# rayandrew/indonesian-image-captioning

Measured on AMD Instinct MI355X. Metric: images/sec (train step, SCN+Attention, bs32/GPU), higher is better.
Workload: dtype f32; 1 GPU; attention_scn decoder (emb/att/factor/dec=512, 1000 tags, V=10000, T=51) + ResNet-152 fine-tune, synthetic tags, bs=32/GPU, 256x256 images, fp32; global_batch=32, parallelism=dp1, call_sequence=harness: encoder(imgs, pooled=False) -> decoder(None, ..., prepool=trunk map)

## Files before the change

include/scnattn.h:

```cpp
#ifndef SCNATTN_H
#define SCNATTN_H

#include <stddef.h>
#include <stdint.h>

#ifdef __cplusplus
extern "C" {
#endif

#define SCNATTN_VERSION 109

int scnattn_version(void);
const char* scnattn_last_error(void);
int scnattn_set_option(const char* name, int value);
int scnattn_profile_collect(double* out6);

typedef struct {
    int B;
    int P;
    int E;
    int A;
    int D;
    int F;
    int M;
// ... 357 lines not shown
    int32_t H, W, C;
    int32_t tab_h;
    int32_t tab_v;
    int32_t reserved;
} scnattn_image_desc;
long scnattn_resize_table_ints(int in_size, int out_size);
int scnattn_u8_resize_bilinear(void* stream, const uint8_t* src, long src_bytes, const scnattn_image_desc* desc_host,
                               const scnattn_image_desc* desc_dev, int N, const int32_t* taps, long taps_len, int OH,
                               int OW, const float* lut, void* dst, int dst_kind, int channels_last);
int scnattn_u8_resize_taps(void* stream, const uint8_t* src, long src_bytes, const scnattn_image_desc* desc_host,
                           const scnattn_image_desc* desc_dev, int N, const int32_t* taps_host, const int32_t* taps_dev,
                           long taps_len, int OH, int OW, const float* lut, void* dst, int dst_kind, int channels_last);
#define SCNATTN_OVERLAY_MAX_MAP 32
#define SCNATTN_OVERLAY_MAX_OUT 1024
int scnattn_attn_strips(int OH);
int scnattn_attn_expand(void* stream, const float* alphas, int n_maps, int h, int w, const float* Mv, const float* Mh,
                        int OH, int OW, float* S, float* lohi, float* partial);
int scnattn_attn_overlay(void* stream, const float* alphas, int n_maps, int h, int w, const float* Mv, const float* Mh,
                         int OH, int OW, const float* S, const float* partial, const uint8_t* img, int n_img,
                         const int32_t* img_index_host, const int32_t* img_index_dev, const float* beta, uint8_t* out);
#define SCNATTN_TEXT_MAX_LEN 128
#define SCNATTN_TEXT_MAX_REFS 32
#define SCNATTN_TEXT_CIDER_MAX_TOKEN 65534
int scnattn_text_max_len(void);
int scnattn_text_ngram_stats(void* stream, int N, int R, const int32_t* hyp, int Lh, const int32_t* hyp_len, const int32_t* ref,
                             int Lr, const int32_t* ref_len, const int32_t* skip_hyp, int n_skip_hyp, const int32_t* skip_ref,
                             int n_skip_ref, int32_t* stats);
int scnattn_text_lcs(void* stream, int N, int R, const int32_t* hyp, int Lh, const int32_t* hyp_len, const int32_t* ref, int Lr,
                     const int32_t* ref_len, const int32_t* skip_hyp, int n_skip_hyp, const int32_t* skip_ref, int n_skip_ref,
                     int32_t* lcs, double* score, double* mean);
int scnattn_text_ref_keys(void* stream, int n, int N, int R, const int32_t* ref, int Lr, const int32_t* ref_len,
                          const int32_t* skip_ref, int n_skip_ref, int64_t* keys, int32_t* flag);
int scnattn_text_cider(void* stream, int N, int R, const int32_t* hyp, int Lh, const int32_t* hyp_len, const int32_t* ref,
                       int Lr, const int32_t* ref_len, const int32_t* skip_hyp, int n_skip_hyp, const int32_t* skip_ref,
                       int n_skip_ref, const int64_t* table_keys, const int32_t* table_df, const long* table_off, long n_images,
                       double* score, double* mean, int32_t* flag);
int scnattn_bn_workspace_floats(int C);
int scnattn_bn_stats(void* stream, int R, int C, const void* x, int bf16, float eps, float momentum, float* partial,
                     float* mean, float* invstd, float* run_mean, float* run_var);
int scnattn_bn_apply(void* stream, int R, int C, const void* z, const void* res, int bf16, const float* mean,
                     const float* invstd, const float* gamma, const float* beta, int relu, void* y);
int scnattn_bn_bwd(void* stream, int R, int C, const void* dy, const void* y, const void* z, int bf16,
                   const float* mean, const float* invstd, const float* gamma, const float* beta, int relu, int train,
                   float* partial, float* dbeta, float* dgamma, void* dz, void* dres);
typedef struct scnattn_conv_extra {
    int pro;
    int epi;
    const float* pro_ss;
    float* stat_partial; const float* stat_shift;
    const float* ez; const float* emean; const float* einvstd; const float* egamma; const float* ebeta; long ldz;
    int stride, Hi, Wi, Ho, Wo;
    int force_split;
    int force_mi;
} scnattn_conv_extra;
int scnattn_cgemm(void* stream, int transA, int transB, int M, int N, int K, float alpha, const float* A, long lda,
                  const float* B, long ldb, float beta, float* C, long ldc, const float* bias, const float* rowmask,
                  int batch, long strideA, long strideB, long strideC, float* ws, long ws_floats,
                  const scnattn_conv_extra* ex);
int scnattn_cgemm_row_tiles(int M);
int scnattn_conv1x1_fwd(void* stream, int R, int Cin, int Cout, const float* x, const float* w, float* y,
                        const scnattn_conv_extra* ex, float* ws, long ws_floats);
int scnattn_conv1x1_dgrad(void* stream, int R, int Cin, int Cout, const float* dy, const float* w, int w_transposed,
                          float beta, float* dx, const scnattn_conv_extra* ex, float* ws, long ws_floats);
int scnattn_conv1x1_wgrad(void* stream, int R, int Cin, int Cout, const float* dy, const float* x, float* dw,
                          const scnattn_conv_extra* ex, float* ws, long ws_floats);
int scnattn_conv3x3_fwd(void* stream, int N, int Hi, int Wi, int Cin, int Cout, int stride, const float* x,
                        const float* w, float* y, const scnattn_conv_extra* ex, float* ws, long ws_floats);
int scnattn_conv3x3_dgrad(void* stream, int N, int Hi, int Wi, int Cin, int Cout, const float* dy, const float* w,
                          float* dx, const scnattn_conv_extra* ex, float* ws, long ws_floats);
int scnattn_conv3x3_dgrad_strided(void* stream, int N, int Hi, int Wi, int Cin, int Cout, int stride, const float* dy,
                                  const float* w, float* dx, float* ws, long ws_floats);
int scnattn_conv3x3_wgrad(void* stream, int N, int Hi, int Wi, int Cin, int Cout, int stride, const float* dy,
                          const float* x, float* dw, float* ws, long ws_floats, int k_slices);
typedef struct scnattn_bn_eval {
    const float* gamma; const float* beta; const float* mean; const float* var; float eps;
    const float* res; long ldres;
    int relu;
} scnattn_bn_eval;
int scnattn_conv1x1_fwd_bn_eval(void* stream, int R, int Cin, int Cout, const float* x, const float* w, float* y,
                                const scnattn_bn_eval* bn, const scnattn_conv_extra* ex, float* ws, long ws_floats);
int scnattn_conv3x3_fwd_bn_eval(void* stream, int N, int Hi, int Wi, int Cin, int Cout, int stride, const float* x,
                                const float* w, float* y, const scnattn_bn_eval* bn, const scnattn_conv_extra* ex,
                                float* ws, long ws_floats);
int scnattn_stem_tiles(int N, int H, int W);
int scnattn_stem_conv7(void* stream, int N, int H, int W, const float* x, long sn, long sc, long sh, long sw,
                       const float* w, long wn, long wc, long wh, long ww, float* z, float* stat_partial,
                       const float* stat_shift);
int scnattn_stem_bn_relu_maxpool(void* stream, int N, int Hz, int Wz, int C, const float* z, const float* ss, void* out,
                                 int out_bf16);
int scnattn_cgemm_stat_ld(int M);
int scnattn_bn_finalize(void* stream, long R, int C, const float* partial, int ldp, int nchunk, const float* shift,
                        float eps, float momentum, float* mean, float* invstd, float* run_mean, float* run_var,
                        const float* gamma, const float* beta, float* ss_out);
int scnattn_bn_apply_fin(void* stream, long R, int C, const void* z, const void* res, int bf16, const float* partial, int ldp,
                         int nchunk, const float* shift, float eps, float momentum, const float* gamma, const float* beta,
                         int relu, void* y, float* mean, float* invstd, float* run_mean, float* run_var, float* ss_out);
int scnattn_bn_bwd_reduce(void* stream, int R, int C, const void* dy, const void* y, const void* z, int bf16, const float* mean,
                          const float* invstd, int relu, float* partial, int ldp_cap, void* gout, int* nchunk_out);
int scnattn_bn_bwd_dx_fin(void* stream, long R, int C, const void* g, const void* z, int bf16, const float* mean,
                          const float* invstd, const float* gamma, const float* partial, int ldp, int nchunk, float* dbeta,
                          float* dgamma, void* dz);

typedef struct scnattn_weight_desc {
    const float* src; void* dst; void* dst_t; int cout, taps, cin, pad;
} scnattn_weight_desc;
int scnattn_bf16_weights(void* stream, int n, const scnattn_weight_desc* desc, const int* tile_prefix, int total_tiles);
int scnattn_cgemm16(void* stream, int M, int N, int K, const void* A, long lda, const void* B, long ldb, float beta, void* C,
                    long ldc, int out_bf16, float* ws, long ws_floats, const scnattn_conv_extra* ex);
int scnattn_conv3x3_fwd16(void* stream, int N, int Hi, int Wi, int Cin, int Cout, int stride, const void* x, const void* w,
                          void* y, const scnattn_conv_extra* ex, float* ws, long ws_floats);
int scnattn_conv3x3_dgrad16(void* stream, int N, int Hi, int Wi, int Cin, int Cout, int stride, const void* dy, const void* wt,
                            void* dx, const scnattn_conv_extra* ex, float* ws, long ws_floats);
typedef struct scnattn_bn_eval16 {
    const float* gamma; const float* beta; const float* mean; const float* var; float eps;
    const void* res; long ldres;
    int relu;
} scnattn_bn_eval16;
int scnattn_conv1x1_fwd_bn_eval16(void* stream, int R, int Cin, int Cout, const void* x, const void* w, void* y,
                                  const scnattn_bn_eval16* bn, const scnattn_conv_extra* ex, float* ws, long ws_floats);
int scnattn_conv3x3_fwd_bn_eval16(void* stream, int N, int Hi, int Wi, int Cin, int Cout, int stride, const void* x,
                                  const void* w, void* y, const scnattn_bn_eval16* bn, const scnattn_conv_extra* ex,
                                  float* ws, long ws_floats);
int scnattn_wgrad16_3x3(void* stream, int N, int H, int W, int Cin, int Cout, const void* dy, const void* x, float* dw,
                        float* ws, long ws_floats, int k_slices);
int scnattn_wgrad16_rows(void* stream, int R, int Cin, int Cout, const void* dy, const void* x, long src_rows, float* dw,
                         long ldo, int gs, int gHi, int gWi, int gHo, int gWo, int goh, int gow, float* ws, long ws_floats,
                         int k_slices);
typedef struct scnattn_block16 {
    int N, Cin, Hi, Wi, p, stride, has_down, pad;
    const float* gamma[4]; const float* beta[4]; float* run_mean[4]; float* run_var[4]; const float* shift[4];
    float eps[4], momentum[4];
    const void* w[4]; const void* wt[4];
    float* ws; long ws_floats; float* part; float* bnpart; long bnpart_floats;
    const void* x; void* save; float* stats;
    const void* dout; void* tmp; float* dgb; float* dw[4]; int need_dx, pad2;
    void* side_stream; float* side_ws; long side_ws_floats;
} scnattn_block16;
int scnattn_block16_sizes(const scnattn_block16* b, long* save_elems, long* out_offset, long* stats_floats, long* tmp_elems,
                          long* dgb_floats);
int scnattn_block16_fwd(void* stream, const scnattn_block16* b);
int scnattn_block16_bwd(void* stream, const scnattn_block16* b, void** dx_out, void** dxd_out);
int scnattn_bn_stats_fold(void* stream, int R, int C, const void* x, float eps, float momentum, float* partial,
                          float* mean, float* invstd, float* run_mean, float* run_var, const float* gamma,
                          const float* beta, float* ss_out);

enum { SCNATTN_PLAN_NONE = 0, SCNATTN_PLAN_CGEMM, SCNATTN_PLAN_SGEMM, SCNATTN_PLAN_SKINNY, SCNATTN_PLAN_CGEMM16,
// ... 48 lines not shown
```

indonesian-image-captioning_amd/csrc/api.cpp:

```cpp
#include <hip/hip_runtime.h>
#include <cstdarg>
#include <cstdio>
#include <cstring>
#include "../../include/scnattn.h"
#include "common.h"
#include "kernels.h"

namespace scn {

static thread_local char g_err[512] = "";

void set_error(const char* fmt, ...) {
    va_list ap;
    va_start(ap, fmt);
    vsnprintf(g_err, sizeof(g_err), fmt, ap);
    va_end(ap);
}
const char* last_error() { return g_err; }

thread_local LaunchPlan* t_plan_out = nullptr;

extern int g_ksplit_scale;
extern int g_profile;
extern int g_attn_depth;
// ... 473 lines not shown
                             const float* enc, float inv_temp, int t0, int n_steps, float* ws) {
    return score_steps(ST(stream), d, K, max_steps, want_alpha, w, enc, inv_temp, t0, n_steps, ws);
}
int scnattn_rollout_score(void* stream, int N, int K, int V, const float* logits, long ld, float inv_temp, int t, int max_steps,
                          void* const* state, const int32_t* target_t, int32_t* rank_t, int32_t* best_t) {
    RolloutState s;
    SCN_TRY(rollout_state_of("scnattn_rollout_score", N, K, max_steps, state, s));
    return rollout_score(ST(stream), N, K, V, logits, ld, inv_temp, t, target_t, rank_t, best_t, s);
}

int scnattn_seq_workspace(const scnattn_dims* d, const scnattn_pool* pool, size_t* saved_bytes, size_t* scratch_bytes) {
    return seq_workspace(d, pool, saved_bytes, scratch_bytes);
}

int scnattn_seq_fwd(void* stream, const scnattn_dims* d, const scnattn_params* w, const float* enc,
                    const float* tags, const int64_t* caps, const int32_t* dl_dev, const int32_t* bt_host,
                    const float* drop_mask, float* saved, float* scratch, float* preds, float* alphas,
                    const scnattn_pool* pool) {
    return seq_fwd(ST(stream), d, w, enc, tags, caps, dl_dev, bt_host, drop_mask, saved, scratch, preds, alphas, pool);
}

int scnattn_seq_bwd(void* stream, const scnattn_dims* d, const scnattn_params* w, const float* enc,
                    const float* tags, const int64_t* caps, const int32_t* dl_dev, const int32_t* bt_host,
                    const float* drop_mask, const float* saved, float* scratch, const float* dpreds,
                    const float* dalphas, const scnattn_params* g, float* denc, float* dtags,
                    const scnattn_pool* pool) {
    return seq_bwd(ST(stream), d, w, enc, tags, caps, dl_dev, bt_host, drop_mask, saved, scratch, dpreds, dalphas, g,
                   denc, dtags, pool);
}

int scnattn_sgemm(void* stream, int transA, int transB, int M, int N, int K, float alpha, const float* A,
                  long lda, const float* B, long ldb, float beta, float* C, long ldc, const float* bias,
                  const float* rowmask, int batch, long strideA, long strideB, long strideC) {
    return sgemm(ST(stream), transA != 0, transB != 0, M, N, K, alpha, A, lda, B, ldb, beta, C, ldc, bias, rowmask,
                 batch < 1 ? 1 : batch, strideA, strideB, strideC);
}

int scnattn_sgemm_ws(void* stream, int transA, int transB, int M, int N, int K, float alpha, const float* A,
                     long lda, const float* B, long ldb, float beta, float* C, long ldc, const float* bias,
                     const float* rowmask, int batch, long strideA, long strideB, long strideC, float* ws,
                     long ws_floats) {
    return sgemm_ws(ST(stream), transA != 0, transB != 0, M, N, K, alpha, A, lda, B, ldb, beta, C, ldc, bias, rowmask,
                    batch < 1 ? 1 : batch, strideA, strideB, strideC, ws, ws ? ws_floats : 0);
}

static ConvExtra to_extra(const scnattn_conv_extra* e) {
    ConvExtra x;
    if (!e) return x;
    x.pro = e->pro; x.epi = e->epi; x.pro_ss = e->pro_ss;
    x.stat_partial = e->stat_partial; x.stat_shift = e->stat_shift;
    x.ez = e->ez; x.emean = e->emean; x.einvstd = e->einvstd; x.egamma = e->egamma; x.ebeta = e->ebeta; x.ldz = e->ldz;
    x.stride = e->stride < 1 ? 1 : e->stride; x.Hi = e->Hi; x.Wi = e->Wi; x.Ho = e->Ho; x.Wo = e->Wo;
    x.force_split = e->force_split; x.force_mi = e->force_mi;
    return x;
}

int scnattn_cgemm(void* stream, int transA, int transB, int M, int N, int K, float alpha, const float* A, long lda,
                  const float* B, long ldb, float beta, float* C, long ldc, const float* bias, const float* rowmask,
                  int batch, long strideA, long strideB, long strideC, float* ws, long ws_floats,
                  const scnattn_conv_extra* ex) {
    const ConvExtra x = to_extra(ex);
    return cgemm(ST(stream), transA != 0, transB != 0, M, N, K, alpha, A, lda, B, ldb, beta, C, ldc, bias, rowmask,
                 batch < 1 ? 1 : batch, strideA, strideB, strideC, ws, ws ? ws_floats : 0, ex ? &x : nullptr);
}

int scnattn_cgemm_row_tiles(int M) { return cgemm_row_tiles(M); }

int scnattn_conv1x1_fwd(void* stream, int R, int Cin, int Cout, const float* x, const float* w, float* y,
                        const scnattn_conv_extra* ex, float* ws, long ws_floats) {
    const ConvExtra e = to_extra(ex);
    SCN_ARG(!ex || ex->pro != 2, "conv1x1_fwd: prologue must be on the input (pro = 1)");
    return cgemm(ST(stream), false, true, R, Cout, Cin, 1.f, x, Cin, w, Cin, 0.f, y, Cout, nullptr, nullptr, 1, 0, 0, 0,
                 ws, ws ? ws_floats : 0, ex ? &e : nullptr);
}

int scnattn_conv1x1_dgrad(void* stream, int R, int Cin, int Cout, const float* dy, const float* w, int w_transposed,
                          float beta, float* dx, const scnattn_conv_extra* ex, float* ws, long ws_floats) {
    const ConvExtra e = to_extra(ex);
    SCN_ARG(!ex || (ex->pro == 0 && ex->stride <= 1), "conv1x1_dgrad: no prologue / stride here");
    if (w_transposed)
        return cgemm(ST(stream), false, true, R, Cin, Cout, 1.f, dy, Cout, w, Cout, beta, dx, Cin, nullptr, nullptr, 1, 0,
                     0, 0, ws, ws ? ws_floats : 0, ex ? &e : nullptr);
    return cgemm(ST(stream), false, false, R, Cin, Cout, 1.f, dy, Cout, w, Cin, beta, dx, Cin, nullptr, nullptr, 1, 0, 0,
                 0, ws, ws ? ws_floats : 0, ex ? &e : nullptr);
}

int scnattn_conv1x1_wgrad(void* stream, int R, int Cin, int Cout, const float* dy, const float* x, float* dw,
                          const scnattn_conv_extra* ex, float* ws, long ws_floats) {
    ConvExtra e = to_extra(ex);
    SCN_ARG(!ex || (ex->pro != 1 && ex->epi == 0), "conv1x1_wgrad: prologue must be on the input (pro = 2), no epilogue");
    return cgemm(ST(stream), true, false, Cout, Cin, R, 1.f, dy, Cout, x, Cin, 0.f, dw, Cin, nullptr, nullptr, 1, 0, 0, 0,
                 ws, ws ? ws_floats : 0, ex ? &e : nullptr);
}

static void set_c3(ConvExtra& e, int mode, int c, int N, int Hi, int Wi, int stride) {
    e.c3 = mode; e.c3c = c;
    e.Hi = Hi; e.Wi = Wi; e.Ho = (Hi - 1) / stride + 1; e.Wo = (Wi - 1) / stride + 1; e.stride = stride;
    e.c3_src_rows = mode == 4 ? (long)N * e.Ho * e.Wo : (long)N * Hi * Wi;
}

int scnattn_conv3x3_fwd(void* stream, int N, int Hi, int Wi, int Cin, int Cout, int stride, const float* x,
                        const float* w, float* y, const scnattn_conv_extra* ex, float* ws, long ws_floats) {
    SCN_ARG(N > 0 && Hi > 0 && Wi > 0 && stride >= 1, "conv3x3_fwd: geometry");
    ConvExtra e = to_extra(ex);
    set_c3(e, 1, Cin, N, Hi, Wi, stride);
    return cgemm(ST(stream), false, true, N * e.Ho * e.Wo, Cout, 9 * Cin, 1.f, x, Cin, w, 9L * Cin, 0.f, y, Cout, nullptr,
                 nullptr, 1, 0, 0, 0, ws, ws ? ws_floats : 0, &e);
}

static int bn_eval_extra(const char* who, int Cin, int Cout, const scnattn_bn_eval* bn, const scnattn_conv_extra* ex,
                         ConvExtra* e) {
    if (!bn) { set_error("%s: invalid argument: bn is NULL", who); return -1; }
    if (ex && (ex->pro != 0 || ex->epi != 0)) { set_error("%s: invalid argument: ex carries geometry only (pro = epi = 0)", who); return -1; }
    if (!(bn->gamma && bn->beta && bn->mean && bn->var)) { set_error("%s: invalid argument: null BatchNorm parameter / statistic", who); return -1; }
    if (Cin <= 0 || Cout <= 0 || Cin % 16 || Cout % 16) { set_error("%s: invalid argument: Cin and Cout must be positive multiples of 16", who); return -1; }
    if (!(aligned16(bn->gamma) && aligned16(bn->beta) && aligned16(bn->mean) && aligned16(bn->var))) {
        set_error("%s: invalid argument: BatchNorm vectors must be 16-byte aligned", who); return -1;
    }
    if (bn->res && (!aligned16(bn->res) || bn->ldres % 4 || bn->ldres < Cout)) {
        set_error("%s: invalid argument: res must be 16-byte aligned with ldres %% 4 == 0 and ldres >= Cout", who); return -1;
    }
    if (ex) {
        e->stride = ex->stride < 1 ? 1 : ex->stride; e->Hi = ex->Hi; e->Wi = ex->Wi; e->Ho = ex->Ho; e->Wo = ex->Wo;
        e->force_split = ex->force_split; e->force_mi = ex->force_mi;
// ... 24 lines not shown
}

int scnattn_conv3x3_dgrad(void* stream, int N, int Hi, int Wi, int Cin, int Cout, const float* dy, const float* w,
                          float* dx, const scnattn_conv_extra* ex, float* ws, long ws_floats) {
    SCN_ARG(N > 0 && Hi > 0 && Wi > 0, "conv3x3_dgrad: geometry");
    ConvExtra e = to_extra(ex);
    set_c3(e, 2, Cout, N, Hi, Wi, 1);
    return cgemm(ST(stream), false, false, N * Hi * Wi, Cin, 9 * Cout, 1.f, dy, Cout, w, 9L * Cin, 0.f, dx, Cin, nullptr,
                 nullptr, 1, 0, 0, 0, ws, ws ? ws_floats : 0, &e);
}

int scnattn_conv3x3_dgrad_strided(void* stream, int N, int Hi, int Wi, int Cin, int Cout, int stride, const float* dy,
                                  const float* w, float* dx, float* ws, long ws_floats) {
    SCN_ARG(N > 0 && Hi > 0 && Wi > 0 && stride == 2 && Hi % 2 == 0 && Wi % 2 == 0, "conv3x3_dgrad_strided: stride 2, even map");
    ConvExtra e;
    set_c3(e, 4, Cout, N, Hi, Wi, 2);
    return cgemm(ST(stream), false, false, N * e.Ho * e.Wo, Cin, 9 * Cout, 1.f, dy, Cout, w, 9L * Cin, 0.f, dx, Cin, nullptr,
                 nullptr, 1, 0, 0, 0, ws, ws ? ws_floats : 0, &e);
}

int scnattn_conv3x3_wgrad(void* stream, int N, int Hi, int Wi, int Cin, int Cout, int stride, const float* dy,
                          const float* x, float* dw, float* ws, long ws_floats, int k_slices) {
    SCN_ARG(N > 0 && Hi > 0 && Wi > 0 && stride >= 1, "conv3x3_wgrad: geometry");
    if (stride == 1 && k_slices >= 0 && conv3x3_wgrad_halo_ok(N, Hi, Wi, Cin, Cout, dy, x, dw))
        return conv3x3_wgrad_halo(ST(stream), N, Hi, Wi, Cin, Cout, dy, x, dw, ws, ws ? ws_floats : 0, k_slices);
    ConvExtra e;
    set_c3(e, 3, Cin, N, Hi, Wi, stride);
    return cgemm(ST(stream), true, false, Cout, 9 * Cin, N * e.Ho * e.Wo, 1.f, dy, Cout, x, Cin, 0.f, dw, 9L * Cin, nullptr,
                 nullptr, 1, 0, 0, 0, ws, ws ? ws_floats : 0, &e);
}

int scnattn_stem_tiles(int N, int H, int W) { return stem_tiles(N, H, W); }

int scnattn_stem_conv7(void* stream, int N, int H, int W, const float* x, long sn, long sc, long sh, long sw,
                       const float* w, long wn, long wc, long wh, long ww, float* z, float* stat_partial,
                       const float* stat_shift) {
    return stem_conv7(ST(stream), N, H, W, x, sn, sc, sh, sw, w, wn, wc, wh, ww, z, stat_partial, stat_shift);
}

int scnattn_stem_bn_relu_maxpool(void* stream, int N, int Hz, int Wz, int C, const float* z, const float* ss, void* out,
                                 int out_bf16) {
    return stem_bn_relu_maxpool(ST(stream), N, Hz, Wz, C, z, ss, out, out_bf16);
}

int scnattn_cgemm_stat_ld(int M) { return cgemm_stat_ld(M); }

int scnattn_bn_finalize(void* stream, long R, int C, const float* partial, int ldp, int nchunk, const float* shift,
                        float eps, float momentum, float* mean, float* invstd, float* run_mean, float* run_var,
                        const float* gamma, const float* beta, float* ss_out) {
    return bn_finalize_t(ST(stream), R, C, partial, ldp, nchunk, shift, eps, momentum, mean, invstd, run_mean, run_var, gamma,
                         beta, ss_out);
}

int scnattn_bn_apply_fin(void* stream, long R, int C, const void* z, const void* res, int bf16, const float* partial, int ldp,
                         int nchunk, const float* shift, float eps, float momentum, const float* gamma, const float* beta,
                         int relu, void* y, float* mean, float* invstd, float* run_mean, float* run_var, float* ss_out) {
    return bn_apply_fin(ST(stream), R, C, z, res, bf16, partial, ldp, nchunk, shift, eps, momentum, gamma, beta, relu, y, mean,
                        invstd, run_mean, run_var, ss_out);
}

int scnattn_bn_bwd_reduce(void* stream, int R, int C, const void* dy, const void* y, const void* z, int bf16, const float* mean,
                          const float* invstd, int relu, float* partial, int ldp_cap, void* gout, int* nchunk_out) {
    return bn_bwd_reduce_t(ST(stream), R, C, dy, y, z, bf16, mean, invstd, relu, partial, ldp_cap, gout, nchunk_out);
}

int scnattn_bn_bwd_dx_fin(void* stream, long R, int C, const void* g, const void* z, int bf16, const float* mean,
                          const float* invstd, const float* gamma, const float* partial, int ldp, int nchunk, float* dbeta,
                          float* dgamma, void* dz) {
    return bn_bwd_dx_fin(ST(stream), R, C, g, z, bf16, mean, invstd, gamma, partial, ldp, nchunk, dbeta, dgamma, dz);
}

int scnattn_cgemm16(void* stream, int M, int N, int K, const void* A, long lda, const void* B, long ldb, float beta, void* C,
                    long ldc, int out_bf16, float* ws, long ws_floats, const scnattn_conv_extra* ex) {
    const ConvExtra x = to_extra(ex);
    return cgemm16(ST(stream), M, N, K, A, lda, B, ldb, beta, C, ldc, out_bf16, ws, ws ? ws_floats : 0, ex ? &x : nullptr, 0);
}

int scnattn_conv3x3_fwd16(void* stream, int N, int Hi, int Wi, int Cin, int Cout, int stride, const void* x, const void* w,
                          void* y, const scnattn_conv_extra* ex, float* ws, long ws_floats) {
    SCN_ARG(N > 0 && Hi > 0 && Wi > 0 && stride >= 1, "conv3x3_fwd16: geometry");
    ConvExtra e = to_extra(ex);
    set_c3(e, 1, Cin, N, Hi, Wi, stride);
    return cgemm16(ST(stream), N * e.Ho * e.Wo, Cout, 9 * Cin, x, Cin, w, 9L * Cin, 0.f, y, Cout, 1, ws, ws ? ws_floats : 0, &e, 0);
}

static int bn_eval16_extra(const char* who, const scnattn_bn_eval16* bn, const scnattn_conv_extra* ex, ConvExtra* e) {
    if (!bn) { set_error("%s: invalid argument: bn is NULL", who); return -1; }
    if (ex && (ex->pro != 0 || ex->epi != 0)) { set_error("%s: invalid argument: ex carries geometry only (pro = epi = 0)", who); return -1; }
    if (ex) {
        e->stride = ex->stride < 1 ? 1 : ex->stride; e->Hi = ex->Hi; e->Wi = ex->Wi; e->Ho = ex->Ho; e->Wo = ex->Wo;
        e->force_split = ex->force_split; e->force_mi = ex->force_mi;
    }
    e->epi = 3;
    e->egamma = bn->gamma; e->ebeta = bn->beta; e->emean = bn->mean; e->evar = bn->var; e->eeps = bn->eps;
    e->ez = (const float*)bn->res; e->ldz = bn->res ? bn->ldres : 0; e->erelu = bn->relu != 0;
    return 0;
}

int scnattn_conv1x1_fwd_bn_eval16(void* stream, int R, int Cin, int Cout, const void* x, const void* w, void* y,
                                  const scnattn_bn_eval16* bn, const scnattn_conv_extra* ex, float* ws, long ws_floats) {
    ConvExtra e;
    SCN_TRY(bn_eval16_extra("conv1x1_fwd_bn_eval16", bn, ex, &e));
    SCN_ARG(R > 0 && Cin > 0 && Cout > 0 && Cin % 8 == 0 && Cout % 8 == 0, "conv1x1_fwd_bn_eval16: R > 0, Cin and Cout positive multiples of 8");
    return cgemm16(ST(stream), R, Cout, Cin, x, Cin, w, Cin, 0.f, y, Cout, 1, ws, ws ? ws_floats : 0, &e, 0);
}

// ... 447 lines not shown
```

indonesian-image-captioning_amd/csrc/batchnorm.hip:

```cpp
#include "tile.h"
#include <climits>
#include <type_traits>

namespace scn {

namespace {

typedef __bf16 bf16x4 __attribute__((ext_vector_type(4)));
template <typename T> struct IO;
template <> struct IO<float> {
    static __device__ __forceinline__ f32x4 ld(const float* p) { return *reinterpret_cast<const f32x4*>(p); }
    static __device__ __forceinline__ void st(float* p, f32x4 v) { *reinterpret_cast<f32x4*>(p) = v; }
    static __device__ __forceinline__ float ld1(const float* p) { return *p; }
};
template <> struct IO<__bf16> {
    static __device__ __forceinline__ f32x4 ld(const __bf16* p) {
        const bf16x4 v = *reinterpret_cast<const bf16x4*>(p);
        return f32x4{(float)v[0], (float)v[1], (float)v[2], (float)v[3]};
    }
    static __device__ __forceinline__ void st(__bf16* p, f32x4 v) {
        *reinterpret_cast<bf16x4*>(p) = bf16x4{(__bf16)v[0], (__bf16)v[1], (__bf16)v[2], (__bf16)v[3]};
    }
    static __device__ __forceinline__ float ld1(const __bf16* p) { return (float)*p; }
};
// ... 186 lines not shown
    }
#pragma unroll
    for (int k = 0; k < 4; ++k) {
        red[rl][0][cl * 4 + k] = sg[k];
        red[rl][1][cl * 4 + k] = sx[k];
    }
    __syncthreads();
    if (threadIdx.x < 128) {
        const int which = threadIdx.x >> 6, cc = threadIdx.x & 63;
        if (blockIdx.x * 64 + cc < C) {
            float v = red[0][which][cc];
#pragma unroll
            for (int i = 1; i < 16; ++i) v += red[i][which][cc];
            if (ldp > 0) partial[((long)which * C + blockIdx.x * 64 + cc) * ldp + blockIdx.y] = v;
            else partial[((long)blockIdx.y * 2 + which) * C + blockIdx.x * 64 + cc] = v;
        }
    }
}

__device__ __forceinline__ void reduce_partials_t(const float* __restrict__ partial, int C, int ldp, int nchunk, int c0,
                                                  float (*out)[64]) {
    const int ch = threadIdx.x >> 2, q = threadIdx.x & 3, c = c0 + ch;
    const __amdgpu_buffer_rsrc_t rs = make_rsrc(partial, (unsigned)(2L * C * ldp * 4));
    float a = 0.f, b = 0.f;
    const unsigned o1 = (unsigned)((long)c * ldp * 4), o2 = (unsigned)(((long)C + c) * ldp * 4);
    for (int i0 = 4 * q; i0 < nchunk; i0 += 64) {
        f32x4 u[4], v[4];
#pragma unroll
        for (int j = 0; j < 4; ++j) {
            const int i = i0 + 16 * j;
            const bool ok = c < C && i < nchunk;
            u[j] = buf_load4(rs, ok ? o1 + (unsigned)i * 4u : OOB_OFF);
            v[j] = buf_load4(rs, ok ? o2 + (unsigned)i * 4u : OOB_OFF);
        }
#pragma unroll
        for (int j = 0; j < 4; ++j) {
            const int i = i0 + 16 * j;
#pragma unroll
            for (int e = 0; e < 4; ++e) {
                a += (i + e < nchunk) ? u[j][e] : 0.f;
                b += (i + e < nchunk) ? v[j][e] : 0.f;
            }
        }
    }
    a += __shfl_xor(a, 1, 64); a += __shfl_xor(a, 2, 64);
    b += __shfl_xor(b, 1, 64); b += __shfl_xor(b, 2, 64);
    if (q == 0) { out[0][ch] = a; out[1][ch] = b; }
    __syncthreads();
}

struct BnFin {
    const float* partial; int ldp, nchunk; const float* shift; float eps, momentum;
    float* mean; float* invstd; float* run_mean; float* run_var; float* ss_out;
};

template <typename T, bool RELU, bool RES>
__global__ __launch_bounds__(256) void bn_apply_fin_kernel(long R, int C, int rows_per_chunk, const T* __restrict__ z,
                                                           const T* __restrict__ res, const float* __restrict__ gamma,
                                                           const float* __restrict__ beta, T* __restrict__ y, BnFin f) {
    __shared__ float st[2][64];
    __shared__ float smu[64], sis[64];
    const int c0 = blockIdx.x * 64;
    const int cl = threadIdx.x & 15, rl = threadIdx.x >> 4, cq = min(c0 + cl * 4, C - 4);
    const long r0 = (long)blockIdx.y * rows_per_chunk, r1 = min(R, r0 + rows_per_chunk);
    f32x4 v[4], rr[4];
    long r = r0 + rl;
#pragma unroll
    for (int j = 0; j < 4; ++j) {
        const long off = min(r + 16 * j, r1 - 1) * C + cq;
        v[j] = IO<T>::ld(z + off);
        if (RES) rr[j] = IO<T>::ld(res + off);
    }
    reduce_partials_t(f.partial, C, f.ldp, f.nchunk, c0, st);
    if (threadIdx.x < 64 && c0 + threadIdx.x < C) {
        const int c = c0 + threadIdx.x;
        const float inv_n = 1.f / (float)R;
        const float m1 = st[0][threadIdx.x] * inv_n;
        const float mu = (f.shift ? f.shift[c] : 0.f) + m1;
        float var = st[1][threadIdx.x] * inv_n - m1 * m1;
        if (var < 0.f) var = 0.f;
        const float is = rsqrtf(var + f.eps);
        smu[threadIdx.x] = mu;
        sis[threadIdx.x] = is;
        if (blockIdx.y == 0) {
            f.mean[c] = mu;
            f.invstd[c] = is;
            if (f.run_mean) f.run_mean[c] = (1.f - f.momentum) * f.run_mean[c] + f.momentum * mu;
            if (f.run_var) {
                const float unbiased = R > 1 ? var * ((float)R / (float)(R - 1)) : var;
                f.run_var[c] = (1.f - f.momentum) * f.run_var[c] + f.momentum * unbiased;
            }
            if (f.ss_out) {
                const float sc = gamma[c] * is;
                f.ss_out[2 * c] = sc;
                f.ss_out[2 * c + 1] = fmaf(-mu, sc, beta[c]);
            }
        }
    }
    __syncthreads();
    const int c = c0 + cl * 4;
    if (c >= C) return;
    const f32x4 mu = *reinterpret_cast<const f32x4*>(smu + cl * 4), is = *reinterpret_cast<const f32x4*>(sis + cl * 4);
    const f32x4 ga = *reinterpret_cast<const f32x4*>(gamma + c), be = *reinterpret_cast<const f32x4*>(beta + c);
    while (r < r1) {
        f32x4 o[4];
#pragma unroll
        for (int j = 0; j < 4; ++j)
#pragma unroll
            for (int k = 0; k < 4; ++k) {
                float t = bn_norm(v[j][k], mu[k], is[k], ga[k], be[k]);
                if (RES) t += rr[j][k];
                if (RELU) t = fmaxf(t, 0.f);
                o[j][k] = t;
            }
        const long rn = r + 64;
        if (rn < r1) {
#pragma unroll
            for (int j = 0; j < 4; ++j) {
                const long off = min(rn + 16 * j, r1 - 1) * C + c;
                v[j] = IO<T>::ld(z + off);
                if (RES) rr[j] = IO<T>::ld(res + off);
            }
        }
#pragma unroll
        for (int j = 0; j < 4; ++j)
            if (r + 16 * j < r1) IO<T>::st(y + (r + 16 * j) * C + c, o[j]);
        r = rn;
    }
}

__global__ __launch_bounds__(256) void bn_finalize_t_kernel(long R, int C, const float* __restrict__ gamma,
                                                            const float* __restrict__ beta, BnFin f) {
    __shared__ float st[2][64];
    const int c0 = blockIdx.x * 64;
    reduce_partials_t(f.partial, C, f.ldp, f.nchunk, c0, st);
    if (threadIdx.x >= 64 || c0 + threadIdx.x >= C) return;
    const int c = c0 + threadIdx.x;
    const float inv_n = 1.f / (float)R;
    const float m1 = st[0][threadIdx.x] * inv_n;
    const float mu = (f.shift ? f.shift[c] : 0.f) + m1;
    float var = st[1][threadIdx.x] * inv_n - m1 * m1;
    if (var < 0.f) var = 0.f;
    const float is = rsqrtf(var + f.eps);
    f.mean[c] = mu;
    f.invstd[c] = is;
    if (f.run_mean) f.run_mean[c] = (1.f - f.momentum) * f.run_mean[c] + f.momentum * mu;
    if (f.run_var) {
        const float unbiased = R > 1 ? var * ((float)R / (float)(R - 1)) : var;
        f.run_var[c] = (1.f - f.momentum) * f.run_var[c] + f.momentum * unbiased;
    }
    if (f.ss_out) {
        const float sc = gamma[c] * is;
        f.ss_out[2 * c] = sc;
        f.ss_out[2 * c + 1] = fmaf(-mu, sc, beta[c]);
    }
}

template <typename T>
__global__ __launch_bounds__(256) void bn_bwd_dx_fin_kernel(long R, int C, int rows_per_chunk, const T* __restrict__ g,
                                                            const T* __restrict__ z, const float* __restrict__ mean,
                                                            const float* __restrict__ invstd, const float* __restrict__ gamma,
                                                            const float* __restrict__ partial, int ldp, int nchunk,
                                                            float* __restrict__ dbeta, float* __restrict__ dgamma,
                                                            T* __restrict__ dz) {
    __shared__ float st[2][64];
    const int c0 = blockIdx.x * 64;
    const int cl = threadIdx.x & 15, rl = threadIdx.x >> 4, c = c0 + cl * 4, cq = min(c, C - 4);
    const long r0 = (long)blockIdx.y * rows_per_chunk, r1 = min(R, r0 + rows_per_chunk);
    f32x4 gg[4], zz[4];
    long r = r0 + rl;
#pragma unroll
    for (int j = 0; j < 4; ++j) {
        const long off = min(r + 16 * j, r1 - 1) * C + cq;
        gg[j] = IO<T>::ld(g + off);
        zz[j] = IO<T>::ld(z + off);
    }
    reduce_partials_t(partial, C, ldp, nchunk, c0, st);
    if (blockIdx.y == 0 && threadIdx.x < 64 && c0 + threadIdx.x < C) {
        dbeta[c0 + threadIdx.x] = st[0][threadIdx.x];
        dgamma[c0 + threadIdx.x] = st[1][threadIdx.x];
    }
    if (c >= C) return;
    const float inv_n = 1.f / (float)R;
    const f32x4 db = *reinterpret_cast<const f32x4*>(&st[0][cl * 4]), dg = *reinterpret_cast<const f32x4*>(&st[1][cl * 4]);
    const f32x4 mu = *reinterpret_cast<const f32x4*>(mean + c), is = *reinterpret_cast<const f32x4*>(invstd + c);
    const f32x4 ga = *reinterpret_cast<const f32x4*>(gamma + c);
    while (r < r1) {
        f32x4 o[4];
#pragma unroll
        for (int j = 0; j < 4; ++j)
#pragma unroll
            for (int k = 0; k < 4; ++k) {
                o[j][k] = bn_dz(gg[j][k], bn_xhat(zz[j][k], mu[k], is[k]), ga[k], is[k], db[k], dg[k], inv_n);
            }
        const long rn = r + 64;
        if (rn < r1) {
#pragma unroll
            for (int j = 0; j < 4; ++j) {
                const long off = min(rn + 16 * j, r1 - 1) * C + c;
                gg[j] = IO<T>::ld(g + off);
                zz[j] = IO<T>::ld(z + off);
            }
        }
#pragma unroll
        for (int j = 0; j < 4; ++j)
            if (r + 16 * j < r1) IO<T>::st(dz + (r + 16 * j) * C + c, o[j]);
        r = rn;
    }
// ... 134 lines not shown
    const bool maskz = relu && !y;
    const bool gfirst = relu && !maskz && dres && dz && sizeof(T) == 4;
    auto reduce = [&](auto RELU, auto MASKZ, auto GOUT) {
        hipLaunchKernelGGL((bn_bwd_reduce_kernel<T, RELU(), MASKZ(), GOUT()>), rgrid, block, 0, st, R, C, rpc, dy, y, z, mean, invstd,
                           gamma, beta, partial, GOUT() ? dres : (T*)nullptr, 0);
    };
    if (maskz) reduce(yes, yes, no);
    else if (relu) on_flag(gfirst, [&](auto GOUT) { reduce(yes, no, GOUT); });
    else reduce(no, no, no);
    SCN_LAUNCH_CHECK();
    hipLaunchKernelGGL(bn_bwd_finalize_kernel, dim3(cdiv(C, 16)), block, 0, st, C, nchunk, partial, dbeta, dgamma);
    SCN_LAUNCH_CHECK();
    if (dz || dres) {
        const long n4 = (long)R * C / 4;
        dim3 grid(ew_blocks(n4));
        const T* g = gfirst ? dres : dy;
        T* dres2 = gfirst ? nullptr : dres;
        on_flag(train, [&](auto TRAIN) {
            auto dx = [&](auto RELU, auto MASKZ) {
                hipLaunchKernelGGL((bn_bwd_dx_kernel<T, RELU(), TRAIN(), MASKZ()>), grid, block, 0, st, n4, R, C, g, y, z, mean, invstd,
                                   gamma, beta, dbeta, dgamma, dz, dres2);
            };
            if (maskz) dx(yes, yes);
            else on_flag(relu && !gfirst, [&](auto RELU) { dx(RELU, no); });
        });
        SCN_LAUNCH_CHECK();
    }
    return 0;
}

int bn_apply_fin(hipStream_t st, long R, int C, const void* z, const void* res, int bf16, const float* partial, int ldp, int nchunk,
                 const float* shift, float eps, float momentum, const float* gamma, const float* beta, int relu, void* y,
                 float* mean, float* invstd, float* run_mean, float* run_var, float* ss_out) {
    SCN_ARG(R > 0 && C > 0 && C % 4 == 0 && z && y && partial && ldp >= nchunk && ldp % 4 == 0 && nchunk > 0 && gamma && beta &&
            mean && invstd && aligned16(partial), "bn_apply_fin: bad argument");
    SCN_ARG(((reinterpret_cast<uintptr_t>(z) | reinterpret_cast<uintptr_t>(y) | reinterpret_cast<uintptr_t>(res)) & (bf16 ? 7u : 15u)) == 0,
            "bn_apply_fin: maps are not vector aligned");
    SCN_ARG(shift != run_mean || !run_mean, "bn_apply_fin: shift must not alias the running mean it updates");
    SCN_ARG(2L * C * ldp * 4 < 0x7fffffffL, "bn_apply_fin: partial too large");
    BnFin f{partial, ldp, nchunk, shift, eps, momentum, mean, invstd, run_mean, run_var, ss_out};
    int rpc;
    const int nch = ew_chunks(R, C, &rpc);
    on_flag(bf16, [&](auto BF) { on_flag(relu, [&](auto RELU) { on_flag(res, [&](auto RES) {
        using T = MapT<BF()>;
        hipLaunchKernelGGL((bn_apply_fin_kernel<T, RELU(), RES()>), dim3(cdiv(C, 64), nch), dim3(256), 0, st, R, C, rpc, (const T*)z,
                           (const T*)res, gamma, beta, (T*)y, f);
    }); }); });
    SCN_LAUNCH_CHECK();
    return 0;
}

int bn_finalize_t(hipStream_t st, long R, int C, const float* partial, int ldp, int nchunk, const float* shift, float eps,
                  float momentum, float* mean, float* invstd, float* run_mean, float* run_var, const float* gamma,
                  const float* beta, float* ss_out) {
    SCN_ARG(R > 0 && C > 0 && partial && ldp >= nchunk && ldp % 4 == 0 && nchunk > 0 && mean && invstd && aligned16(partial),
            "bn_finalize_t: bad argument");
    SCN_ARG(!ss_out || (gamma && beta), "bn_finalize_t: folded scale/shift need gamma and beta");
    SCN_ARG(2L * C * ldp * 4 < 0x7fffffffL, "bn_finalize_t: partial too large");
    BnFin f{partial, ldp, nchunk, shift, eps, momentum, mean, invstd, run_mean, run_var, ss_out};
    hipLaunchKernelGGL(bn_finalize_t_kernel, dim3(cdiv(C, 64)), dim3(256), 0, st, R, C, gamma, beta, f);
    SCN_LAUNCH_CHECK();
    return 0;
}

int bn_bwd_reduce_t(hipStream_t st, int R, int C, const void* dy, const void* y, const void* z, int bf16, const float* mean,
                    const float* invstd, int relu, float* partial, int ldp_cap, void* gout, int* nchunk_out) {
    SCN_ARG(R > 0 && C > 0 && C % 4 == 0 && dy && z && mean && invstd && partial && (!relu || y), "bn_bwd_reduce_t: bad argument");
    SCN_ARG(relu || !gout, "bn_bwd_reduce_t: without relu g is dy itself, gout must be NULL");
    int rpc;
    const int nchunk = pick_chunks(R, C, &rpc);
    const int ldp = (nchunk + 3) & ~3;
    SCN_ARG(ldp <= ldp_cap, "bn_bwd_reduce_t: partial buffer too small");
    const float* nf = nullptr;
    on_flag(bf16, [&](auto BF) {
        using T = MapT<BF()>;
        auto reduce = [&](auto RELU, auto GOUT) {
            hipLaunchKernelGGL((bn_bwd_reduce_kernel<T, RELU(), false, GOUT()>), dim3(cdiv(C, 64), nchunk), dim3(256), 0, st, R, C, rpc,
                               (const T*)dy, (const T*)y, (const T*)z, mean, invstd, nf, nf, partial, (T*)gout, ldp);
        };
        if (relu) on_flag(gout, [&](auto GOUT) { reduce(yes, GOUT); });
        else reduce(no, no);
    });
    SCN_LAUNCH_CHECK();
    if (nchunk_out) *nchunk_out = nchunk;
    return 0;
}

int bn_bwd_dx_fin(hipStream_t st, long R, int C, const void* g, const void* z, int bf16, const float* mean, const float* invstd,
                  const float* gamma, const float* partial, int ldp, int nchunk, float* dbeta, float* dgamma, void* dz) {
    SCN_ARG(R > 0 && C > 0 && C % 4 == 0 && g && z && mean && invstd && gamma && partial && ldp >= nchunk && ldp % 4 == 0 &&
            nchunk > 0 && dbeta && dgamma && dz && aligned16(partial), "bn_bwd_dx_fin: bad argument");
    SCN_ARG(((reinterpret_cast<uintptr_t>(g) | reinterpret_cast<uintptr_t>(z) | reinterpret_cast<uintptr_t>(dz)) & (bf16 ? 7u : 15u)) == 0,
            "bn_bwd_dx_fin: maps are not vector aligned");
    SCN_ARG(2L * C * ldp * 4 < 0x7fffffffL, "bn_bwd_dx_fin: partial too large");
    int rpc;
    const int nch = ew_chunks(R, C, &rpc);
    on_flag(bf16, [&](auto BF) {
        using T = MapT<BF()>;
        hipLaunchKernelGGL(bn_bwd_dx_fin_kernel<T>, dim3(cdiv(C, 64), nch), dim3(256), 0, st, R, C, rpc, (const T*)g, (const T*)z, mean,
                           invstd, gamma, partial, ldp, nchunk, dbeta, dgamma, (T*)dz);
    });
    SCN_LAUNCH_CHECK();
    return 0;
}

int bn_bwd(hipStream_t st, int R, int C, const void* dy, const void* y, const void* z, int bf16, const float* mean,
           const float* invstd, const float* gamma, const float* beta, int relu, int train, float* partial, float* dbeta,
           float* dgamma, void* dz, void* dres) {
    SCN_ARG(R > 0 && C > 0 && C % 4 == 0 && dy && z && mean && invstd && gamma && partial && dbeta && dgamma,
            "bn_bwd: bad argument");
    SCN_ARG(!relu || y || beta, "bn_bwd: relu needs the forward output y, or beta to recompute the mask from z");
    if (bf16) return bn_bwd_t<__bf16>(st, R, C, (const __bf16*)dy, (const __bf16*)y, (const __bf16*)z, mean, invstd, gamma, beta, relu,
// ... 7 lines not shown
```

indonesian-image-captioning_amd/csrc/cgemm.hip:

```cpp
#include "tile.h"
#include <map>
#include <mutex>
#include <type_traits>
#include <utility>

namespace scn {

int cgemm_stat_ld(int M);

namespace {

constexpr int TN = 128, TK = 16, NSTAGE = 3;
constexpr int TILE_F = 128 * TK;
constexpr int AUX_F = 4 * 64;
constexpr int STAGE_F = 2 * TILE_F + AUX_F;
constexpr int SROWS = 64;

struct CArgs {
    const float* A; const float* B; float* C;
    const float* bias; const float* rowmask;
    long lda, ldb, ldc, sA, sB, sC;
    int M, N, K;
    float alpha, beta;
    int S, kper;
    float* ws;
    int mt, nt;
    ConvGeom geo;
    const float* pro_ss;
    float* stat_partial; const float* stat_shift;
    int ldp;
    const float* ez; const float* emean; const float* einvstd; const float* egamma; const float* ebeta;
    long ldz;
    const float* evar; float eeps; int erelu;
    int* cnt;
    int comb;
};

template <int MI, bool A_MC, bool B_MC, int PRO, int EPI, bool GATHER, bool VEC, int C3 = 0>
__global__ __launch_bounds__(256, MI == 2 ? 2 : 3) void cgemm_kernel(CArgs g) {
    __shared__ __attribute__((aligned(16))) float lds[NSTAGE * STAGE_F];
    constexpr bool W41 = (MI == 4);
    constexpr int RB = W41 ? 1 : MI;
    constexpr int TM = W41 ? 128 : 64 * MI;
    constexpr int ACH = TM / 64;
    constexpr int LPT = ACH + 2 + (PRO == 1 ? 1 : 0);

    const int tid = threadIdx.x, lane = tid & 63, wave = tid >> 6;
    const int wm = W41 ? wave : wave >> 1, wn = W41 ? 0 : wave & 1;
    const int hh = lane >> 5, l31 = lane & 31;

    const int ntiles = g.mt * g.nt;
    const int bid = xcd_order(blockIdx.x, ntiles);
    const int tm = bid / g.nt, tn = bid - tm * g.nt;
    const int m0 = tm * TM, n0 = tn * (W41 ? 64 : TN);
    const int cls = C3 == 4 ? 3 - (int)blockIdx.y : 0, ph = cls >> 1, pw = cls & 1, ntw = 1 + pw;
    const int zb = C3 == 4 ? 0 : blockIdx.y / g.S, sp = C3 == 4 ? 0 : blockIdx.y - zb * g.S;
    const float* A = g.A + (long)zb * g.sA;
    const float* B = g.B + (long)zb * g.sB;
    float* C = g.C + (long)zb * g.sC;
    const int kbeg = sp * g.kper, Kend = C3 == 4 ? (1 + ph) * ntw * g.geo.c3c : min(g.K, kbeg + g.kper);
    const int nk = (Kend - kbeg + TK - 1) / TK;

    const long a_elems = (C3 == 1 || C3 == 2 || C3 == 4) ? g.geo.src_rows * g.lda
                         : A_MC ? ((long)(g.K - 1) * g.lda + g.M)
                                : (GATHER ? (gather_row(g.geo, g.M - 1) * g.lda + g.K) : ((long)(g.M - 1) * g.lda + g.K));
    const long b_elems = C3 == 3 ? g.geo.src_rows * g.ldb
                         : (C3 == 2 || C3 == 4) ? (long)(g.K / 9) * g.ldb
                         : B_MC ? ((GATHER && A_MC ? gather_row(g.geo, g.K - 1) : (long)(g.K - 1)) * g.ldb + g.N)
                                : ((long)(g.N - 1) * g.ldb + g.K);
    const __amdgpu_buffer_rsrc_t ars = make_rsrc(A, (unsigned)(a_elems * 4));
    const __amdgpu_buffer_rsrc_t brs = make_rsrc(B, (unsigned)(b_elems * 4));
    const __amdgpu_buffer_rsrc_t srs = make_rsrc(g.pro_ss, PRO == 1 ? (unsigned)g.K * 8u : 0u);

    unsigned a_off[ACH], b_off[2];
    bool a_ok[ACH], b_ok[2];
    int a_nb[ACH], a_h0[ACH], a_w0[ACH];
#pragma unroll
    for (int c = 0; c < ACH; ++c) {
        const int chunk = wave * ACH + c;
        if (C3 == 1 || C3 == 2 || C3 == 4) {
            const int row = chunk * 16 + (lane >> 2), gsrc = (lane & 3) ^ ((row >> 2) & 3);
            const int grow = m0 + row;
            a_ok[c] = grow < g.M;
            const Pixel p = pixel_of(a_ok[c] ? grow : 0, g.geo.Ho, g.geo.Wo);
            a_nb[c] = p.n * g.geo.Hi * g.geo.Wi;
            a_h0[c] = C3 == 4 ? p.h : p.h * g.geo.s - 1;
            a_w0[c] = C3 == 4 ? p.w : p.w * g.geo.s - 1;
            a_off[c] = (unsigned)(gsrc * 16);
        } else if (!A_MC) {
            const int row = chunk * 16 + (lane >> 2), gsrc = (lane & 3) ^ ((row >> 2) & 3);
            const int grow = m0 + row;
            a_ok[c] = grow < g.M;
            const long src = (GATHER ? gather_row(g.geo, a_ok[c] ? grow : 0) : (long)grow) * g.lda + gsrc * 4;
            a_off[c] = (unsigned)(src * 4);
        } else if (TM == 128) {
            const int col = m0 + 4 * (lane & 31);
            a_ok[c] = col < g.M;
            a_off[c] = (unsigned)(((long)(chunk * 2 + (lane >> 5)) * g.lda + col) * 4);
        } else {
            const int col = m0 + 4 * (lane & 15);
            a_ok[c] = col < g.M;
            a_off[c] = (unsigned)(((long)(chunk * 4 + (lane >> 4)) * g.lda + col) * 4);
        }
    }
#pragma unroll
    for (int c = 0; c < 2; ++c) {
        const int chunk = wave * 2 + c;
        if (!B_MC) {
            const int row = chunk * 16 + (lane >> 2), gsrc = (lane & 3) ^ ((row >> 2) & 3);
            const int grow = n0 + row;
            b_ok[c] = grow < g.N && (!W41 || row < 64);
            b_off[c] = (unsigned)(((long)grow * g.ldb + gsrc * 4) * 4);
        } else {
            const int col = n0 + 4 * (lane & 31);
            b_ok[c] = col < g.N && (!W41 || (lane & 31) < 16);
            b_off[c] = (unsigned)(((long)(chunk * 2 + (lane >> 5)) * g.ldb + col) * 4);
        }
    }

    auto issue_piece = [&](int kt, int stage, auto pc) {
        constexpr int P = decltype(pc)::value;
        float* sa = lds + stage * STAGE_F;
        float* sb = sa + TILE_F;
        const int k0 = kbeg + kt * TK;
        if constexpr (P < ACH) {
            constexpr int c = P;
            const int chunk = wave * ACH + c;
            unsigned va;
            if (C3 == 4) {
                const int t = k0 / g.geo.c3c, c0 = k0 - t * g.geo.c3c, th = t / ntw, tw = t - th * ntw;
                const int hi = a_h0[c] + ((ph && th == 0) ? 1 : 0), wi = a_w0[c] + ((pw && tw == 0) ? 1 : 0);
                const bool ok = a_ok[c] && k0 < Kend && hi < g.geo.Hi && wi < g.geo.Wi;
                va = ok ? (unsigned)(((long)(a_nb[c] + hi * g.geo.Wi + wi) * g.lda + c0) * 4) + a_off[c] : OOB_OFF;
            } else if (C3 == 1 || C3 == 2) {
                const int tap = k0 / g.geo.c3c, c0 = k0 - tap * g.geo.c3c;
                int dh = tap / 3, dw = tap - 3 * dh;
                if (C3 == 2) { dh = 2 - dh; dw = 2 - dw; }
                const int hi = a_h0[c] + dh, wi = a_w0[c] + dw;
                const bool ok = a_ok[c] && k0 < Kend && (unsigned)hi < (unsigned)g.geo.Hi && (unsigned)wi < (unsigned)g.geo.Wi;
                va = ok ? (unsigned)(((long)(a_nb[c] + hi * g.geo.Wi + wi) * g.lda + c0) * 4) + a_off[c] : OOB_OFF;
            } else if (!A_MC) {
                const int kk = k0 + 4 * ((lane & 3) ^ (((chunk * 16 + (lane >> 2)) >> 2) & 3));
                va = (a_ok[c] && kk < Kend) ? a_off[c] + (unsigned)k0 * 4u : OOB_OFF;
            } else {
                const int kr = k0 + (TM == 128 ? chunk * 2 + (lane >> 5) : chunk * 4 + (lane >> 4));
                va = (a_ok[c] && kr < Kend) ? a_off[c] + (unsigned)((long)k0 * g.lda * 4) : OOB_OFF;
            }
            dma16(ars, sa + chunk * 256, va);
        }
        if constexpr (P >= ACH && P < ACH + 2) {
            constexpr int c = P - ACH;
            const int chunk = wave * 2 + c;
            unsigned vb;
            if (!B_MC) {
                const int kk = k0 + 4 * ((lane & 3) ^ (((chunk * 16 + (lane >> 2)) >> 2) & 3));
                vb = (b_ok[c] && kk < Kend) ? b_off[c] + (unsigned)k0 * 4u : OOB_OFF;
            } else {
                const int kr = k0 + chunk * 2 + (lane >> 5);
                if (C3 == 4) {
                    const int t = k0 / g.geo.c3c, co = kr - t * g.geo.c3c, th = t / ntw, tw = t - th * ntw;
                    const int tap = (ph ? 2 * th : 1) * 3 + (pw ? 2 * tw : 1);
                    vb = (b_ok[c] && kr < Kend) ? (unsigned)(((long)co * g.ldb + (long)tap * g.N + n0 + 4 * (lane & 31)) * 4) : OOB_OFF;
                } else if (C3 == 2) {
                    const int tap = k0 / g.geo.c3c, co = kr - tap * g.geo.c3c;
                    vb = (b_ok[c] && kr < Kend) ? (unsigned)(((long)co * g.ldb + (long)tap * g.N + n0 + 4 * (lane & 31)) * 4) : OOB_OFF;
                } else if (C3 == 3) {
                    const int tap = n0 / g.geo.c3c, ci0 = n0 - tap * g.geo.c3c, dh = tap / 3, dw = tap - 3 * dh;
                    const Pixel p = pixel_of(kr < Kend ? kr : 0, g.geo.Ho, g.geo.Wo);
                    const int n = p.n, hi = p.h * g.geo.s + dh - 1, wi = p.w * g.geo.s + dw - 1;
                    const bool ok = b_ok[c] && kr < Kend && (unsigned)hi < (unsigned)g.geo.Hi && (unsigned)wi < (unsigned)g.geo.Wi;
                    vb = ok ? (unsigned)(((long)(n * g.geo.Hi * g.geo.Wi + hi * g.geo.Wi + wi) * g.ldb + ci0 + 4 * (lane & 31)) * 4) : OOB_OFF;
                } else if (GATHER && A_MC) {
                    const long src = gather_row(g.geo, kr < Kend ? kr : 0) * g.ldb + n0 + 4 * (lane & 31);
                    vb = (b_ok[c] && kr < Kend) ? (unsigned)(src * 4) : OOB_OFF;
                } else {
                    vb = (b_ok[c] && kr < Kend) ? b_off[c] + (unsigned)((long)k0 * g.ldb * 4) : OOB_OFF;
                }
            }
            dma16(brs, sb + chunk * 256, vb);
        }
        if constexpr (PRO == 1 && P == ACH + 2) {
            float* sx = sa + 2 * TILE_F + wave * 64;
            const int kk = k0 + (lane >> 1);
            dma4(srs, sx, (lane < 32 && kk < Kend) ? (unsigned)(2 * k0 + lane) * 4u : OOB_OFF);
        }
    };

    auto issue = [&](int kt, int stage) {
        issue_piece(kt, stage, std::integral_constant<int, 0>{});
        if constexpr (LPT > 1) issue_piece(kt, stage, std::integral_constant<int, 1>{});
        if constexpr (LPT > 2) issue_piece(kt, stage, std::integral_constant<int, 2>{});
        if constexpr (LPT > 3) issue_piece(kt, stage, std::integral_constant<int, 3>{});
        if constexpr (LPT > 4) issue_piece(kt, stage, std::integral_constant<int, 4>{});
    };

    f32x16 acc[RB][2];
#pragma unroll
    for (int i = 0; i < RB; ++i)
#pragma unroll
        for (int j = 0; j < 2; ++j)
#pragma unroll
            for (int r = 0; r < 16; ++r) acc[i][j][r] = 0.f;

    float bsc[2] = {1.f, 1.f}, bsh[2] = {0.f, 0.f};
    if (PRO == 2) {
#pragma unroll
        for (int j = 0; j < 2; ++j) {
            const int n = n0 + wn * 64 + j * 32 + l31;
            if (n < g.N) { bsc[j] = g.pro_ss[2 * n]; bsh[j] = g.pro_ss[2 * n + 1]; }
        }
#pragma unroll
        for (int j = 0; j < 2; ++j) { asm volatile("" : "+v"(bsc[j])); asm volatile("" : "+v"(bsh[j])); }
    }

    auto prologue_in_lds = [&](int stg) {
        float* sa = lds + stg * STAGE_F;
        const float* sx = sa + 2 * TILE_F + wave * 64;
#pragma unroll
        for (int c = 0; c < ACH; ++c) {
            const int chunk = wave * ACH + c;
            const int row = chunk * 16 + (lane >> 2), gsrc = (lane & 3) ^ ((row >> 2) & 3);
            float* p = sa + chunk * 256 + lane * 4;
            f32x4 v = *reinterpret_cast<f32x4*>(p);
            const f32x4 t0 = *reinterpret_cast<const f32x4*>(sx + 8 * gsrc), t1 = *reinterpret_cast<const f32x4*>(sx + 8 * gsrc + 4);
            v[0] = fmaxf(fmaf(v[0], t0[0], t0[1]), 0.f);
            v[1] = fmaxf(fmaf(v[1], t0[2], t0[3]), 0.f);
            v[2] = fmaxf(fmaf(v[2], t1[0], t1[1]), 0.f);
            v[3] = fmaxf(fmaf(v[3], t1[2], t1[3]), 0.f);
            *reinterpret_cast<f32x4*>(p) = v;
        }
        asm volatile("s_waitcnt lgkmcnt(0)" ::: "memory");
    };

    auto load_piece = [&](int stg, auto pc, float (&a)[RB][8], float (&b)[2][8]) {
        constexpr int P = decltype(pc)::value;
        const float* sa = lds + stg * STAGE_F;
        const float* sb = sa + TILE_F;
        if constexpr (P < RB) {
            constexpr int i = P;
            if (!A_MC) {
                const int row = wm * 32 * RB + i * 32 + l31, sw = (row >> 2) & 3;
                const f32x4 v0 = *reinterpret_cast<const f32x4*>(sa + row * 16 + (((2 * hh) ^ sw) << 2));
                const f32x4 v1 = *reinterpret_cast<const f32x4*>(sa + row * 16 + (((2 * hh + 1) ^ sw) << 2));
#pragma unroll
                for (int q = 0; q < 4; ++q) { a[i][q] = v0[q]; a[i][4 + q] = v1[q]; }
            } else {
                const int col = wm * 32 * RB + i * 32 + l31;
#pragma unroll
                for (int q = 0; q < 8; ++q) a[i][q] = sa[(8 * hh + q) * TM + col];
            }
        } else {
            constexpr int j = P - RB;
            if (!B_MC) {
                const int row = wn * 64 + j * 32 + l31, sw = (row >> 2) & 3;
                const f32x4 v0 = *reinterpret_cast<const f32x4*>(sb + row * 16 + (((2 * hh) ^ sw) << 2));
                const f32x4 v1 = *reinterpret_cast<const f32x4*>(sb + row * 16 + (((2 * hh + 1) ^ sw) << 2));
#pragma unroll
                for (int q = 0; q < 4; ++q) { b[j][q] = v0[q]; b[j][4 + q] = v1[q]; }
            } else {
                const int col = wn * 64 + j * 32 + l31;
#pragma unroll
                for (int q = 0; q < 8; ++q) b[j][q] = sb[(8 * hh + q) * 128 + col];
            }
        }
    };
    auto load_frags = [&](int stg, float (&a)[RB][8], float (&b)[2][8]) {
        load_piece(stg, std::integral_constant<int, 0>{}, a, b);
        load_piece(stg, std::integral_constant<int, 1>{}, a, b);
        load_piece(stg, std::integral_constant<int, 2>{}, a, b);
        if constexpr (RB == 2) load_piece(stg, std::integral_constant<int, 3>{}, a, b);
    };
    auto slot = [](int kt) { return kt % NSTAGE; };
    [[maybe_unused]] f32x4 pv[ACH], pt0[ACH], pt1[ACH];
    auto pro_read = [&](int stg) {
        const float* sa = lds + stg * STAGE_F;
        const float* sx = sa + 2 * TILE_F + wave * 64;
#pragma unroll
        for (int c = 0; c < ACH; ++c) {
            const int chunk = wave * ACH + c;
            const int row = chunk * 16 + (lane >> 2), gsrc = (lane & 3) ^ ((row >> 2) & 3);
            pv[c] = *reinterpret_cast<const f32x4*>(sa + chunk * 256 + lane * 4);
            pt0[c] = *reinterpret_cast<const f32x4*>(sx + 8 * gsrc);
            pt1[c] = *reinterpret_cast<const f32x4*>(sx + 8 * gsrc + 4);
        }
    };
    auto pro_apply = [&](int stg) {
        float* sa = lds + stg * STAGE_F;
#pragma unroll
        for (int c = 0; c < ACH; ++c) {
            const int chunk = wave * ACH + c;
            f32x4 v = pv[c];
            v[0] = fmaxf(fmaf(v[0], pt0[c][0], pt0[c][1]), 0.f);
            v[1] = fmaxf(fmaf(v[1], pt0[c][2], pt0[c][3]), 0.f);
            v[2] = fmaxf(fmaf(v[2], pt1[c][0], pt1[c][1]), 0.f);
            v[3] = fmaxf(fmaf(v[3], pt1[c][2], pt1[c][3]), 0.f);
            *reinterpret_cast<f32x4*>(sa + chunk * 256 + lane * 4) = v;
        }
    };
    constexpr int NPL = RB + 2, NM = 16 * RB;
    constexpr int NPC = NPL + LPT + (PRO == 1 ? 2 : 0);
    float fa0[RB][8], fb0[2][8], fa1[RB][8], fb1[2][8];
    auto kstep = [&](int kt, float (&ac)[RB][8], float (&bc)[2][8], float (&an)[RB][8], float (&bn)[2][8]) {
        const int s_next = slot(kt + 1), s_dma = slot(kt), s_pro = slot(kt + 2);
        auto piece = [&](auto pc) {
            constexpr int P = decltype(pc)::value;
            if constexpr (PRO != 1) {
                if constexpr (P < NPL) load_piece(s_next, pc, an, bn);
                else if constexpr (P < NPC) issue_piece(kt + 3, s_dma, std::integral_constant<int, P - NPL>{});
            } else {
                if constexpr (P < LPT) issue_piece(kt + 3, s_dma, pc);
                else if constexpr (P == LPT) { wait_vmcnt<LPT>(); pro_read(s_pro); }
                else if constexpr (P < LPT + 1 + NPL) load_piece(s_next, std::integral_constant<int, P - LPT - 1>{}, an, bn);
                else if constexpr (P < NPC) pro_apply(s_pro);
            }
        };
        if (PRO == 2) {
#pragma unroll
            for (int j = 0; j < 2; ++j)
#pragma unroll
                for (int q = 0; q < 8; ++q) bc[j][q] = fmaxf(fmaf(bc[j][q], bsc[j], bsh[j]), 0.f);
        }
#pragma unroll
        for (int q = 0; q < 8; ++q)
#pragma unroll
            for (int i = 0; i < RB; ++i)
#pragma unroll
                for (int j = 0; j < 2; ++j) {
                    const int m = (q * RB + i) * 2 + j;
                    acc[i][j] = __builtin_amdgcn_mfma_f32_32x32x2f32(ac[i][q], bc[j][q], acc[i][j], 0, 0, 0);
                    if (m == 0 * NM / NPC) piece(std::integral_constant<int, 0>{});
                    if (m == 1 * NM / NPC) piece(std::integral_constant<int, 1>{});
                    if (m == 2 * NM / NPC) piece(std::integral_constant<int, 2>{});
                    if (m == 3 * NM / NPC) piece(std::integral_constant<int, 3>{});
                    if (m == 4 * NM / NPC) piece(std::integral_constant<int, 4>{});
                    if (m == 5 * NM / NPC) piece(std::integral_constant<int, 5>{});
                    if (m == 6 * NM / NPC) piece(std::integral_constant<int, 6>{});
                    if (m == 7 * NM / NPC) piece(std::integral_constant<int, 7>{});
                    if (m == 8 * NM / NPC) piece(std::integral_constant<int, 8>{});
                    if (m == 9 * NM / NPC) piece(std::integral_constant<int, 9>{});
                    if (m == 10 * NM / NPC) piece(std::integral_constant<int, 10>{});
                    __builtin_amdgcn_sched_barrier(0);
                }
        static_assert(NPC <= 11 && NPC <= NM, "more pieces than slots");
        if (PRO != 1) wait_vmcnt<LPT>();
        __builtin_amdgcn_s_waitcnt(0xC07F);
        __builtin_amdgcn_s_barrier();
    };

    issue(0, 0);
    issue(1, 1);
    issue(2, 2);
    asm volatile("s_waitcnt vmcnt(%0)" :: "n"(2 * LPT) : "memory");
    if (PRO == 1) prologue_in_lds(0);
    __builtin_amdgcn_s_barrier();
    load_frags(0, fa0, fb0);
    wait_vmcnt<LPT>();
    if (PRO == 1) prologue_in_lds(1);
    __builtin_amdgcn_s_waitcnt(0xC07F);
    __builtin_amdgcn_s_barrier();
    for (int kt = 0; kt < nk; kt += 2) {
        kstep(kt, fa0, fb0, fa1, fb1);
        if (kt + 1 < nk) kstep(kt + 1, fa1, fb1, fa0, fb0);
    }
    wait_vmcnt<0>();
    __builtin_amdgcn_s_barrier();

    unsigned opq = 0;
    asm volatile("" : "+v"(opq));
    float* const lw = lds + wave * 2048;
    float* const colsum = lds + 4 * 2048;
    const int rl = lane >> 4, c4 = (lane & 15) * 4;
    const int ncol = n0 + wn * 64 + c4;
    const bool cok = ncol < g.N;
    const long c_ld = g.S > 1 ? (long)g.N : g.ldc;
    float* const c_base = g.S > 1 ? g.ws + ((long)blockIdx.y * g.M) * g.N : C;
    const __amdgpu_buffer_rsrc_t ors = make_rsrc(c_base, VEC ? (unsigned)(((long)((C3 == 4 ? 4 * g.M : g.M) - 1) * c_ld + g.N) * 4) : 0u);
    auto row_off = [&](int m) -> unsigned {
        if (!(m < g.M && cok)) return OOB_OFF;
        const long rr = C3 == 4 ? class_row_scatter(g.geo, m, ph, pw) : m;
        return (unsigned)((rr * c_ld + ncol) * 4) + opq;
    };
    auto dump_half = [&](int i, float add0, float add1) {
#pragma unroll
        for (int j = 0; j < 2; ++j)
#pragma unroll
            for (int r = 0; r < 16; ++r)
                lw[mfma32_row(r, lane) * 64 + j * 32 + l31] = g.alpha * acc[i][j][r] + (j ? add1 : add0);
        asm volatile("s_waitcnt lgkmcnt(0)" ::: "memory");
    };
    const int mw0 = m0 + wm * 32 * RB;

    [[maybe_unused]] f32x4 kv0 = {0.f, 0.f, 0.f, 0.f}, kv1 = kv0, kv2 = kv0, kv3 = kv0;
    const bool folded = EPI == 2 && g.pro_ss != nullptr;
    [[maybe_unused]] float fs1[4] = {0.f, 0.f, 0.f, 0.f}, fs2[4] = {0.f, 0.f, 0.f, 0.f};
    [[maybe_unused]] f32x4 xv[8];
    [[maybe_unused]] float mk[8];
    const bool f_use_c = EPI == 0 && g.beta != 0.f, f_use_m = EPI == 0 && g.rowmask != nullptr;
    const __amdgpu_buffer_rsrc_t f_crs = make_rsrc(C, VEC ? (unsigned)(((long)(g.M - 1) * g.ldc + g.N) * 4) : 0u);
    const bool f_use_r = EPI == 2 || (EPI == 3 && g.ez != nullptr);
    const __amdgpu_buffer_rsrc_t f_zrs = make_rsrc(g.ez, (VEC && f_use_r) ? (unsigned)(((long)(g.M - 1) * g.ldz + g.N) * 4) : 0u);
    const __amdgpu_buffer_rsrc_t f_mrs = make_rsrc(g.rowmask, f_use_m ? (unsigned)g.M * 4u : 0u);
    auto out_off = [&](int m) -> unsigned { return (m < g.M && cok) ? (unsigned)(((long)m * g.ldc + ncol) * 4) + opq : OOB_OFF; };
    auto finish_setup = [&]() {
        if (!cok) return;
        if (EPI == 0 && g.bias) kv0 = *reinterpret_cast<const f32x4*>(g.bias + ncol);
        if (EPI == 1 && g.stat_shift) kv0 = *reinterpret_cast<const f32x4*>(g.stat_shift + ncol);
        if (EPI == 2) {
            kv0 = *reinterpret_cast<const f32x4*>(g.emean + ncol);
            kv1 = *reinterpret_cast<const f32x4*>(g.einvstd + ncol);
            if (folded) {
// ... 516 lines not shown
    int* p = nullptr;
    if (hipMalloc(&p, CNT_N * sizeof(int)) != hipSuccess) return nullptr;
    if (hipMemset(p, 0, CNT_N * sizeof(int)) != hipSuccess || hipDeviceSynchronize() != hipSuccess) { (void)hipFree(p); return nullptr; }
    g_cnt[{dev, st}] = p;
    return p;
}
}

bool cgemm_supported(bool tA, bool tB, int M, int N, int K, const float* A, long lda, const float* B, long ldb,
                     long sA, long sB) {
    if (!(aligned16(A) && aligned16(B) && lda % 4 == 0 && ldb % 4 == 0 && sA % 4 == 0 && sB % 4 == 0 && K >= 1)) return false;
    if (!tA && K % 4) return false;
    if (tA && M % 4) return false;
    if (tB && K % 4) return false;
    if (!tB && N % 4) return false;
    const long abytes = (tA ? ((long)(K - 1) * lda + M) : ((long)(M - 1) * lda + K)) * 4;
    const long bbytes = (tB ? ((long)(N - 1) * ldb + K) : ((long)(K - 1) * ldb + N)) * 4;
    return abytes < 0x7fffffffL && bbytes < 0x7fffffffL;
}

namespace {

template <int MI, bool AMC, bool BMC, int PRO, bool G>
void launch_ev(hipStream_t st, dim3 grid, const CArgs& g, const LaunchPlan& p) {
    dim3 block(256);
    if (p.epi == 2) {
        if constexpr (!AMC && BMC && PRO == 0 && !G) hipLaunchKernelGGL((cgemm_kernel<MI, false, true, 0, 2, false, true>), grid, block, 0, st, g);
    } else if (p.epi == 3) {
        if constexpr (!AMC && !BMC && PRO == 0) hipLaunchKernelGGL((cgemm_kernel<MI, false, false, 0, 3, G, true>), grid, block, 0, st, g);
    } else if (p.epi == 1) hipLaunchKernelGGL((cgemm_kernel<MI, AMC, BMC, PRO, 1, G, true>), grid, block, 0, st, g);
    else if (p.vec) hipLaunchKernelGGL((cgemm_kernel<MI, AMC, BMC, PRO, 0, G, true>), grid, block, 0, st, g);
    else            hipLaunchKernelGGL((cgemm_kernel<MI, AMC, BMC, PRO, 0, G, false>), grid, block, 0, st, g);
}

template <int MI>
void launch_conv3(hipStream_t st, dim3 grid, const CArgs& g, const LaunchPlan& p) {
    dim3 block(256);
    if (p.c3 == 1) {
        if (p.epi == 1) hipLaunchKernelGGL((cgemm_kernel<MI, false, false, 0, 1, false, true, 1>), grid, block, 0, st, g);
        else if (p.epi == 3) hipLaunchKernelGGL((cgemm_kernel<MI, false, false, 0, 3, false, true, 1>), grid, block, 0, st, g);
        else            hipLaunchKernelGGL((cgemm_kernel<MI, false, false, 0, 0, false, true, 1>), grid, block, 0, st, g);
    } else if (p.c3 == 2) {
        if (p.epi == 2) hipLaunchKernelGGL((cgemm_kernel<MI, false, true, 0, 2, false, true, 2>), grid, block, 0, st, g);
        else            hipLaunchKernelGGL((cgemm_kernel<MI, false, true, 0, 0, false, true, 2>), grid, block, 0, st, g);
    } else if (p.c3 == 4) {
        hipLaunchKernelGGL((cgemm_kernel<MI, false, true, 0, 0, false, true, 4>), grid, block, 0, st, g);
    } else {
        hipLaunchKernelGGL((cgemm_kernel<MI, true, true, 0, 0, false, true, 3>), grid, block, 0, st, g);
    }
}

template <int MI>
void launch_layout(hipStream_t st, dim3 grid, const CArgs& g, const LaunchPlan& p) {
    if (!p.tA && p.tB) {
        if (p.gather) { if (p.pro == 1) launch_ev<MI, false, false, 1, true>(st, grid, g, p); else launch_ev<MI, false, false, 0, true>(st, grid, g, p); }
        else          { if (p.pro == 1) launch_ev<MI, false, false, 1, false>(st, grid, g, p); else launch_ev<MI, false, false, 0, false>(st, grid, g, p); }
    } else if (!p.tA && !p.tB) {
        launch_ev<MI, false, true, 0, false>(st, grid, g, p);
    } else if (p.tA && !p.tB) {
        if (p.gather) { if (p.pro == 2) launch_ev<MI, true, true, 2, true>(st, grid, g, p); else launch_ev<MI, true, true, 0, true>(st, grid, g, p); }
        else          { if (p.pro == 2) launch_ev<MI, true, true, 2, false>(st, grid, g, p); else launch_ev<MI, true, true, 0, false>(st, grid, g, p); }
    } else {
        launch_ev<MI, true, false, 0, false>(st, grid, g, p);
    }
}

struct CgemmFacts {
    int pro, epi, c3;
    bool gather, vec;
    int force_mi, force_split;
    bool ws;
    long ws_floats;
};

int cgemm_plan(LaunchPlan& p, bool tA, bool tB, int M, int N, int K, int batch, const CgemmFacts& f, bool counters_ok) {
    const int c3 = f.c3, epi = f.epi;
    int mi = 2;
    if ((long)cdiv(M, 128) * cdiv(N, TN) * batch < 256 && M > 64 && c3 != 1 && c3 != 2 && c3 != 4) mi = 1;
    if (c3 == 4 && (long)cdiv(M, 128) * cdiv(N, TN) * 4 < 768) mi = 1;
    if (N <= 64 && M >= 128 && c3 != 3) mi = 4;
    if (g_cgemm_mi == 1 || g_cgemm_mi == 2) mi = g_cgemm_mi;
    if (f.force_mi > 0) mi = f.force_mi;
    SCN_ARG(mi == 1 || mi == 2 || (mi == 4 && c3 != 3), "cgemm: bad tile selector");
    const int nt = cdiv(N, mi == 4 ? 64 : TN);
    const int tmrows = mi == 4 ? 128 : 64 * mi, mt = cdiv(M, tmrows);
    const long tiles = (long)mt * nt * batch;
    int S = 1;
    if (f.ws && tiles < 224 && K >= 2 * g_cgemm_kmin) {
        long target = g_cgemm_target;
        if (g_cgemm_target == 512) {
            if (c3 == 3) target = 768;
            else if (!tA && K >= 4096 && !c3) target = 1100;
        }
        S = (int)((target + tiles - 1) / tiles);
        const int smax = K / g_cgemm_kmin;
        if (S > smax) S = smax;
        if (S > CG_MAX_SPLIT) S = CG_MAX_SPLIT;
        while (S > 1 && (long)S * batch * M * N > f.ws_floats) --S;
        if (S < 1) S = 1;
    }
    if (f.ws && !c3 && S == 1 && tiles >= 224 && tiles < 768 && K >= 1536 && g_cgemm_target == 512) {
        S = (int)((1200 + tiles / 2) / tiles);
        const int smax = K / (2 * g_cgemm_kmin);
        if (S > smax) S = smax;
        while (S > 1 && (long)S * batch * M * N > f.ws_floats) --S;
        if (S < 1) S = 1;
    }
    if (c3 == 4) S = 1;
    if ((c3 == 1 || c3 == 2) && f.ws) {
        S = (int)(512 / (tiles > 0 ? tiles : 1));
        if (S > 4) S = 4;
        if (S < 1) S = 1;
        while (S > 1 && (long)S * M * N > f.ws_floats) --S;
    }
    if (f.force_split > 0 && c3 != 4) {
        S = f.force_split;
        SCN_ARG(S == 1 || (f.ws && (long)S * batch * M * N <= f.ws_floats && S <= CG_MAX_SPLIT), "cgemm: forced split does not fit");
    }
    const bool comb_ok = g_cgemm_combine && f.vec && tiles <= CNT_N && counters_ok;
    if (epi == 3 && S > 1) {
        if (S > g_cgemm_combine_max) S = g_cgemm_combine_max;
        if (!(comb_ok && S > 1 && (long)S * M * N * 4 < 0x7fffffffL)) S = 1;
    }
    int kper = cdiv(K, S);
    kper = (kper + TK - 1) / TK * TK;
    S = cdiv(K, kper);
    const bool epi_in = epi != 2 || (!tA && !tB && f.pro == 0 && !f.gather && c3 == 0) || c3 == 2;
    const bool in_launch = S > 1 && comb_ok && S <= g_cgemm_combine_max && epi_in && (epi == 0 || !tA) &&
                           (long)S * M * N * 4 < 0x7fffffffL;
    SCN_ARG(epi != 3 || S == 1 || in_launch, "cgemm: eval BatchNorm epilogue of a split product needs the in-launch combine");
    const int kepi = (S > 1 && !in_launch) ? 0 : (epi_in ? epi : 0);
    if (c3) SCN_ARG(f.vec, "cgemm: 3x3 mode needs 16-byte row stores");
    else if (!tA && !tB) SCN_ARG(!f.gather && f.pro == 0, "cgemm: NN product takes no gather / prologue");
    else if (tA && !tB) SCN_ARG(kepi == 0, "cgemm: TN product takes no statistics epilogue");
    else if (tA && tB) SCN_ARG(!f.gather && f.pro == 0 && kepi == 0, "cgemm: TT product is plain");
    p = LaunchPlan{};
    p.family = SCNATTN_PLAN_CGEMM;
    p.mi = mi; p.tA = tA; p.tB = tB; p.pro = f.pro; p.epi = kepi; p.gather = f.gather; p.c3 = c3; p.vec = f.vec;
    p.S = S; p.kper = kper; p.mt = mt; p.nt = nt; p.tiles = tiles;
    p.grid_x = mt * nt; p.grid_y = c3 == 4 ? 4 : batch * S; p.grid_z = 1;
    p.in_launch = in_launch;
    if ((S > 1 && !in_launch) || (epi == 2 && !epi_in))
        p.second = epi == 0 ? SCNATTN_SECOND_CREDUCE : epi == 1 ? SCNATTN_SECOND_CSTATS1
                   : S == 1 ? SCNATTN_SECOND_CSTATS2_C : SCNATTN_SECOND_CSTATS2_SLABS;
    return 0;
}

}

int cgemm(hipStream_t st, bool tA, bool tB, int M, int N, int K, float alpha, const float* A, long lda, const float* B,
          long ldb, float beta, float* C, long ldc, const float* bias, const float* rowmask, int batch, long sA, long sB,
          long sC, float* ws, long ws_floats, const ConvExtra* ex) {
    const PlanQuery query;
    if (M <= 0 || N <= 0 || batch <= 0) return 0;
    SCN_ARG(A && B && C, "cgemm: null operand");
    SCN_ARG(cgemm_supported(tA, tB, M, N, K, A, lda, B, ldb, sA, sB), "cgemm: operand alignment / size not supported");
    SCN_ARG(beta == 0.f || ((long)(M - 1) * ldc + N) * 4 < 0x7fffffffL, "cgemm: C too large for beta != 0");
    const int pro = ex ? ex->pro : 0, epi = ex ? ex->epi : 0;
    const int c3 = ex ? ex->c3 : 0;
    const bool gather = ex && ex->stride > 1 && c3 == 0;
    if (c3) {
        SCN_ARG(c3 >= 1 && c3 <= 4 && pro == 0 && batch == 1 && beta == 0.f && !bias && !rowmask, "cgemm: 3x3 mode takes a plain product");
        SCN_ARG(ex->Hi > 0 && ex->Wi > 0 && ex->Ho > 0 && ex->Wo > 0 && ex->stride >= 1 && ex->c3c > 0 && ex->c3_src_rows > 0, "cgemm: 3x3 geometry");
        SCN_ARG((c3 == 1 && !tA && tB && K == 9 * ex->c3c && ex->c3c % 16 == 0) ||
                (c3 == 2 && !tA && !tB && K == 9 * ex->c3c && ex->c3c % 16 == 0 && ex->stride == 1) ||
                (c3 == 4 && !tA && !tB && K == 9 * ex->c3c && ex->c3c % 16 == 0 && ex->stride == 2 && epi == 0 &&
                 ex->Hi == 2 * ex->Ho && ex->Wi == 2 * ex->Wo && (long)4 * M * ldc * 4 < 0x7fffffffL) ||
                (c3 == 3 && tA && !tB && N == 9 * ex->c3c && ex->c3c % 128 == 0), "cgemm: 3x3 mode / layout / channel multiple");
        SCN_ARG(ex->c3_src_rows * (c3 == 3 ? ldb : lda) * 4 < 0x7fffffffL, "cgemm: 3x3 source map exceeds the descriptor range");
    }
    SCN_ARG(pro == 0 || (pro == 1 && !tA) || (pro == 2 && !tB && tA), "cgemm: prologue / layout mismatch");
    SCN_ARG(epi == 0 || (batch == 1 && beta == 0.f && !bias && !rowmask && (epi == 3 || ex->stat_partial)),
            "cgemm: statistics epilogue needs a plain product");
    SCN_ARG(epi != 3 || (!tA && tB && pro == 0 && (c3 == 0 || c3 == 1)), "cgemm: eval BatchNorm epilogue: forward products only");
    SCN_ARG(epi != 3 || (ex->egamma && ex->ebeta && ex->emean && ex->evar && aligned16(ex->egamma) && aligned16(ex->ebeta) &&
                         aligned16(ex->emean) && aligned16(ex->evar) &&
                         (!ex->ez || (aligned16(ex->ez) && ex->ldz % 4 == 0 && ex->ldz >= N &&
                                      ((long)(M - 1) * ex->ldz + N) * 4 < 0x7fffffffL))),
            "cgemm: eval BatchNorm epilogue arguments");
    SCN_ARG(epi != 2 || (ex->ez && ex->emean && ex->einvstd && (ex->pro_ss || (ex->egamma && ex->ebeta)) && ex->ldz % 4 == 0),
            "cgemm: mask epilogue arguments");
    SCN_ARG(pro == 0 || ex->pro_ss, "cgemm: prologue table");
    SCN_ARG(!gather || (ex->Hi > 0 && ex->Wi > 0 && ex->Ho > 0 && ex->Wo > 0 && batch == 1), "cgemm: gather geometry");
    const bool vec = N % 4 == 0 && ldc % 4 == 0 && sC % 4 == 0 && aligned16(C) &&
                     ((long)(M - 1) * ldc + N) * 4 < 0x7fffffffL && (long)M * N * 4 < 0x7fffffffL;
    SCN_ARG(epi == 0 || vec, "cgemm: the statistics epilogues need N % 4 == 0, ldc % 4 == 0 and a 16-byte aligned C");

    const CgemmFacts f{pro, epi, c3, gather, vec, ex ? ex->force_mi : 0, ex ? ex->force_split : 0, ws != nullptr, ws_floats};
    LaunchPlan p;
    SCN_TRY(cgemm_plan(p, tA, tB, M, N, K, batch, f, true));
    if (query.answer(p)) return 0;
    int* cnt = nullptr;
    if (p.in_launch && !(cnt = stream_counters(st)))
        SCN_TRY(cgemm_plan(p, tA, tB, M, N, K, batch, f, false));

    CArgs g{};
    g.A = A; g.B = B; g.C = C; g.bias = bias; g.rowmask = rowmask;
    g.lda = lda; g.ldb = ldb; g.ldc = ldc; g.sA = sA; g.sB = sB; g.sC = sC;
    g.M = M; g.N = N; g.K = K; g.alpha = alpha; g.beta = beta; g.S = p.S; g.kper = p.kper; g.ws = ws; g.mt = p.mt; g.nt = p.nt;
    if (ex) {
        g.geo = conv_geom(*ex);
        g.pro_ss = ex->pro_ss;
        g.stat_partial = ex->stat_partial; g.stat_shift = ex->stat_shift; g.ldp = cgemm_stat_ld(M);
        g.ez = ex->ez; g.emean = ex->emean; g.einvstd = ex->einvstd; g.egamma = ex->egamma; g.ebeta = ex->ebeta; g.ldz = ex->ldz;
        g.evar = ex->evar; g.eeps = ex->eeps; g.erelu = ex->erelu;
    }
    g.cnt = cnt; g.comb = g_cgemm_combine;
    const dim3 grid(p.grid_x, p.grid_y), block(256);
    if (p.c3) {
        if (p.mi == 4) launch_conv3<4>(st, grid, g, p);
        else if (p.mi == 2) launch_conv3<2>(st, grid, g, p);
        else launch_conv3<1>(st, grid, g, p);
    } else if (p.mi == 4) launch_layout<4>(st, grid, g, p);
    else if (p.mi == 2) launch_layout<2>(st, grid, g, p);
    else launch_layout<1>(st, grid, g, p);
    SCN_LAUNCH_CHECK();
    if (p.second) {
        if (p.second == SCNATTN_SECOND_CREDUCE) {
            if (p.vec) hipLaunchKernelGGL(creduce_kernel<true>, dim3(cdiv((long)M * N / 4, 256), batch), block, 0, st, g);
            else       hipLaunchKernelGGL(creduce_kernel<false>, dim3(cdiv((long)M * N, 256), batch), block, 0, st, g);
        } else {
            if (p.second == SCNATTN_SECOND_CSTATS2_C) g.S = 0;
            dim3 sgrid(cdiv(N, 64), cdiv(M, SROWS));
            if (p.second == SCNATTN_SECOND_CSTATS1) hipLaunchKernelGGL(cstats_kernel<1>, sgrid, block, 0, st, g);
            else                                    hipLaunchKernelGGL(cstats_kernel<2>, sgrid, block, 0, st, g);
        }
        SCN_LAUNCH_CHECK();
    }
    return 0;
}

int cgemm_row_tiles(int M) { return cdiv(M, SROWS); }
int cgemm_stat_ld(int M) { return (cdiv(M, SROWS) + 3) & ~3; }

int cgemm_reduce(hipStream_t st, const float* ws, int S, int M, int N, float* C, long ldc) {
    SCN_ARG(ws && C && S >= 1 && M > 0 && N > 0 && N % 4 == 0 && ldc % 4 == 0 && aligned16(ws) && aligned16(C),
            "cgemm_reduce: arguments");
    CArgs g{};
    g.ws = const_cast<float*>(ws); g.C = C; g.M = M; g.N = N; g.S = S; g.ldc = ldc;
    hipLaunchKernelGGL(creduce_kernel<true>, dim3(cdiv((long)M * N / 4, 256), 1), dim3(256), 0, st, g);
    SCN_LAUNCH_CHECK();
    return 0;
}

}
```

indonesian-image-captioning_amd/csrc/kernels.h:

```cpp
#pragma once
#include <hip/hip_runtime.h>

#include "../../include/scnattn.h"

#define SCN_MAX_KSPLIT 16

namespace scn {

typedef ::scnattn_launch_plan LaunchPlan;
extern thread_local LaunchPlan* t_plan_out;
struct PlanQuery {
    LaunchPlan* out;
    PlanQuery() : out(t_plan_out) { if (out) { t_plan_out = nullptr; *out = LaunchPlan{}; } }
    bool answer(const LaunchPlan& p) const { if (out) *out = p; return out != nullptr; }
    void hand_on() const { t_plan_out = out; }
};

int sgemm(hipStream_t st, bool tA, bool tB, int M, int N, int K, float alpha, const float* A, long lda,
          const float* B, long ldb, float beta, float* C, long ldc, const float* bias,
          const float* rowmask, int batch, long sA, long sB, long sC);

int sgemm_ws(hipStream_t st, bool tA, bool tB, int M, int N, int K, float alpha, const float* A, long lda,
             const float* B, long ldb, float beta, float* C, long ldc, const float* bias, const float* rowmask,
             int batch, long sA, long sB, long sC, float* ws, long ws_floats);

struct ConvExtra {
    int pro = 0;
    int epi = 0;
    const float* pro_ss = nullptr;
    float* stat_partial = nullptr;
    const float* stat_shift = nullptr;
    const float* ez = nullptr; const float* emean = nullptr; const float* einvstd = nullptr;
    const float* egamma = nullptr; const float* ebeta = nullptr; long ldz = 0;
    int stride = 1, Hi = 0, Wi = 0, Ho = 0, Wo = 0;
    int force_split = 0;
    int force_mi = 0;
    int c3 = 0;
    int c3c = 0;
    long c3_src_rows = 0;
    const float* evar = nullptr; float eeps = 0.f; int erelu = 0;
};
bool cgemm_supported(bool tA, bool tB, int M, int N, int K, const float* A, long lda, const float* B, long ldb,
                     long sA, long sB);
int cgemm(hipStream_t st, bool tA, bool tB, int M, int N, int K, float alpha, const float* A, long lda, const float* B,
          long ldb, float beta, float* C, long ldc, const float* bias, const float* rowmask, int batch, long sA, long sB,
          long sC, float* ws, long ws_floats, const ConvExtra* ex);
int cgemm_row_tiles(int M);
int cgemm_stat_ld(int M);
int cgemm_reduce(hipStream_t st, const float* ws, int S, int M, int N, float* C, long ldc);

bool conv3x3_wgrad_halo_ok(int N, int H, int W, int C, int Co, const float* dy, const float* x, const float* dw);
int conv3x3_wgrad_halo(hipStream_t st, int N, int H, int W, int C, int Co, const float* dy, const float* x, float* dw,
                       float* ws, long ws_floats, int force_split);

int stem_tiles(int N, int H, int W);
int stem_conv7(hipStream_t st, int N, int H, int W, const float* x, long sn, long sc, long sh, long sw, const float* w,
               long wn, long wc, long wh, long ww, float* z, float* partial, const float* stat_shift);
int stem_bn_relu_maxpool(hipStream_t st, int N, int Hz, int Wz, int C, const float* z, const float* ss, void* out, int out_bf16);

int skinny_pick_ksplit(int rows, int N, int K, int groups);
struct Slabs {
    const float* p; int n; long stride; long ld;
};
int skinny_gemm(hipStream_t st, int rows, int N, int K, int groups, const float* X, long ldx, long xg,
                const void* W, long ldw, long wg, float* Y, long ldy, long yg, long yslab, int ksplit, int wbf = 0);

int attn_scores(hipStream_t st, int rows, int P, int A, const void* att1, Slabs att2, const float* bd,
                const float* w, const float* b0, float* e, float* att2_out, bool bf = false);
int attn_context(hipStream_t st, int rows, int P, int E, const void* enc, const float* e, Slabs gpre,
                 const float* bbeta, float* alpha_out, long alpha_ld, float* alpha_save, float* awe,
                 float* gate, float* z, bool bf = false);
int mean_pixels(hipStream_t st, int rows, int P, int E, const float* enc, float* out);
struct PoolDesc {
    int Q, qtap_max;
    const int* tap_idx;
    const float* tap_w;
    const int* qtap_idx;
    const float* qtap_w;
    const float* col_w;
};
int pool_desc(const ::scnattn_pool* p, PoolDesc& out);
int attn_context_pooled(hipStream_t st, int rows, int P, int E, const void* x, const PoolDesc& pool, const float* e,
                        Slabs gpre, const float* bbeta, float* alpha_out, long alpha_ld, float* alpha_save,
                        float* alphaq_save, float* awe, float* gate, float* z, bool bf = false);
int weighted_rows(hipStream_t st, int rows, int Q, int E, const float* x, const float* wts, float* out);
int attn_softmax_bwd_pooled(hipStream_t st, int rows, int P, int A, const void* att1, const float* att2, const float* w,
                            const float* alpha, const PoolDesc& pool, const float* dalphaq, const float* dalpha_in,
                            long dalpha_in_ld, float* de, float* datt2, long datt2_ld, bool bf = false);
int pool_expand(hipStream_t st, int B, int P, int A, const PoolDesc& pool, const float* y, const float* bias, float* out);
int pool_transpose(hipStream_t st, int B, int P, int A, const PoolDesc& pool, const float* in, float* out);
int add_bcast_rows_w(hipStream_t st, int B, int Q, int E, const float* wts, const float* v, float* out);
int attn_dalpha(hipStream_t st, int rows, int P, int E, const void* enc, const float* dawe,
                const float* dalpha_in, long dalpha_in_ld, float* dalpha, bool bf = false);
// ... 143 lines not shown
            float* rows, float* out);
int bce_bwd(hipStream_t st, int B, int S, const float* probs, long ldp, const float* t, long ldt, const float* g, float* dz,
            long lddz);
int u8_gather_normalize(hipStream_t st, const uint8_t* src, long n_src, const long long* idx, long n_out, int C,
                        long HW, const float* lut, void* dst, int dst_bf16, int channels_last);
int u8_resize_bilinear(hipStream_t st, const uint8_t* src, long src_bytes, const struct scnattn_image_desc* desc_host,
                       const struct scnattn_image_desc* desc_dev, int N, const int* taps, long taps_len, int OH, int OW,
                       const float* lut, void* dst, int dst_kind, int channels_last);
long resize_table_ints(int in, int out);
int u8_resize_taps(hipStream_t st, const uint8_t* src, long src_bytes, const struct scnattn_image_desc* desc_host,
                   const struct scnattn_image_desc* desc_dev, int N, const int* taps_host, const int* taps_dev,
                   long taps_len, int OH, int OW, const float* lut, void* dst, int dst_kind, int channels_last);
int attn_expand(hipStream_t st, const float* alphas, int n_maps, int h, int w, const float* Mv, const float* Mh, int OH,
                int OW, float* S, float* lohi, float* partial);
int attn_overlay(hipStream_t st, const float* alphas, int n_maps, int h, int w, const float* Mv, const float* Mh, int OH,
                 int OW, const float* S, const float* partial, const uint8_t* img, int n_img, const int* idx_host,
                 const int* idx_dev, const float* beta, uint8_t* out);
int attn_strips(int OH);
int text_max_len();
int text_ngram_stats(hipStream_t st, int N, int R, const int32_t* hyp, int Lh, const int32_t* hyp_len, const int32_t* ref,
                     int Lr, const int32_t* ref_len, const int32_t* skip_hyp, int n_skip_hyp, const int32_t* skip_ref,
                     int n_skip_ref, int32_t* stats);
int text_lcs(hipStream_t st, int N, int R, const int32_t* hyp, int Lh, const int32_t* hyp_len, const int32_t* ref, int Lr,
             const int32_t* ref_len, const int32_t* skip_hyp, int n_skip_hyp, const int32_t* skip_ref, int n_skip_ref,
             int32_t* lcs, double* score, double* mean);
int text_ref_keys(hipStream_t st, int n, int N, int R, const int32_t* ref, int Lr, const int32_t* ref_len,
                  const int32_t* skip_ref, int n_skip_ref, int64_t* keys, int32_t* flag);
int text_cider(hipStream_t st, int N, int R, const int32_t* hyp, int Lh, const int32_t* hyp_len, const int32_t* ref, int Lr,
               const int32_t* ref_len, const int32_t* skip_hyp, int n_skip_hyp, const int32_t* skip_ref, int n_skip_ref,
               const int64_t* table_keys, const int32_t* table_df, const long* table_off, long n_images, double* score,
               double* mean, int32_t* flag);
int pool_permute_fwd(hipStream_t st, int B, int C, int Hin, int Win, int Ho, int Wo, const float* x,
                     long sxb, long sxc, long sxh, long sxw, float* y);
int pool_permute_bwd(hipStream_t st, int B, int C, int Hin, int Win, int Ho, int Wo, const float* dy,
                     float* dx, long sxb, long sxc, long sxh, long sxw);
int clamp_adam(hipStream_t st, long n, float* p, const float* g, float* m, float* v, double lr, double b1,
               double b2, double eps, int step, double clip, double gscale);
int mul_bcast(hipStream_t st, int T, int B, int N, const float* x, const float* q, float* out);
int reduce_slabs(hipStream_t st, int rows, int N, Slabs s, float* out);
int f32_to_bf16(hipStream_t st, long n, const float* in, void* out);

int bn_max_chunks();
int bn_stats(hipStream_t st, int R, int C, const void* x, int bf16, float eps, float momentum, float* partial,
             float* mean, float* invstd, float* run_mean, float* run_var, const float* gamma = nullptr,
             const float* beta = nullptr, float* ss_out = nullptr);
int bn_apply(hipStream_t st, int R, int C, const void* z, const void* res, int bf16, const float* mean,
             const float* invstd, const float* gamma, const float* beta, int relu, void* y);
int bn_bwd(hipStream_t st, int R, int C, const void* dy, const void* y, const void* z, int bf16, const float* mean,
           const float* invstd, const float* gamma, const float* beta, int relu, int train, float* partial, float* dbeta,
           float* dgamma, void* dz, void* dres);

int bn_finalize_t(hipStream_t st, long R, int C, const float* partial, int ldp, int nchunk, const float* shift, float eps,
                  float momentum, float* mean, float* invstd, float* run_mean, float* run_var, const float* gamma,
                  const float* beta, float* ss_out);
int bn_apply_fin(hipStream_t st, long R, int C, const void* z, const void* res, int bf16, const float* partial, int ldp, int nchunk,
                 const float* shift, float eps, float momentum, const float* gamma, const float* beta, int relu, void* y,
                 float* mean, float* invstd, float* run_mean, float* run_var, float* ss_out);
int bn_bwd_reduce_t(hipStream_t st, int R, int C, const void* dy, const void* y, const void* z, int bf16, const float* mean,
                    const float* invstd, int relu, float* partial, int ldp_cap, void* gout, int* nchunk_out);
int bn_bwd_dx_fin(hipStream_t st, long R, int C, const void* g, const void* z, int bf16, const float* mean, const float* invstd,
                  const float* gamma, const float* partial, int ldp, int nchunk, float* dbeta, float* dgamma, void* dz);

int cgemm16(hipStream_t st, int M, int N, int K, const void* A, long lda, const void* B, long ldb, float beta, void* C, long ldc,
            int out_bf16, float* ws, long ws_floats, const ConvExtra* ex, int flip);
int wgrad16_3x3(hipStream_t st, int N, int H, int W, int C, int Co, const void* dy, const void* x, float* dw, float* ws,
                long ws_floats, int force_split);
int wgrad16_rows(hipStream_t st, int R, int C, int Co, const void* dy, const void* x, long src_rows, float* dw, long ldo,
                 int gs, int gHi, int gWi, int gHo, int gWo, int goh, int gow, float* ws, long ws_floats, int force_split);
struct WeightDesc { const float* src; void* dst; void* dst_t; int cout, taps, cin, pad; };
int bf16_weights(hipStream_t st, int n, const WeightDesc* desc, const int* tile_prefix, int total_tiles);

}
```

indonesian-image-captioning_amd/scnattn/_lib.py:

```python
import ctypes as C
import os
import threading

import torch

_HERE = os.path.dirname(os.path.abspath(__file__))
LIB_PATH = os.path.join(_HERE, "libscnattn.so")

_lib = None
_lock = threading.Lock()

vp, i32, i64, f32, f64, sz = C.c_void_p, C.c_int, C.c_long, C.c_float, C.c_double, C.c_size_t


class Dims(C.Structure):
    _fields_ = [(n, C.c_int) for n in ("B", "P", "E", "A", "D", "F", "M", "S", "V", "T", "L", "has_att")]


PARAM_FIELDS = (
    "attention_encoder_att_weight", "attention_encoder_att_bias",
    "attention_decoder_att_weight", "attention_decoder_att_bias",
    "attention_full_att_weight", "attention_full_att_bias",
    "embedding_weight",
    "decode_step_weight_ia", "decode_step_weight_ib", "decode_step_weight_ic",
    "decode_step_weight_ha", "decode_step_weight_hb", "decode_step_weight_hc",
    "decode_step_bias_ih", "decode_step_bias_hh",
    "init_h_weight", "init_h_bias", "init_c_weight", "init_c_bias",
    "f_beta_weight", "f_beta_bias", "fc_weight", "fc_bias",
)


class Params(C.Structure):
    _fields_ = [(n, C.c_void_p) for n in PARAM_FIELDS]


class Pool(C.Structure):
    _fields_ = [("Q", C.c_int), ("qtap_max", C.c_int), ("tap_idx", C.c_void_p), ("tap_w", C.c_void_p),
                ("qtap_idx", C.c_void_p), ("qtap_w", C.c_void_p), ("col_w", C.c_void_p)]


class ConvExtra(C.Structure):
    _fields_ = [("pro", C.c_int), ("epi", C.c_int), ("pro_ss", C.c_void_p),
                ("stat_partial", C.c_void_p), ("stat_shift", C.c_void_p), ("ez", C.c_void_p), ("emean", C.c_void_p),
                ("einvstd", C.c_void_p), ("egamma", C.c_void_p), ("ebeta", C.c_void_p), ("ldz", C.c_long),
                ("stride", C.c_int), ("Hi", C.c_int), ("Wi", C.c_int), ("Ho", C.c_int), ("Wo", C.c_int),
                ("force_split", C.c_int), ("force_mi", C.c_int)]


class BnEval(C.Structure):
    _fields_ = [("gamma", C.c_void_p), ("beta", C.c_void_p), ("mean", C.c_void_p), ("var", C.c_void_p), ("eps", C.c_float),
                ("res", C.c_void_p), ("ldres", C.c_long), ("relu", C.c_int)]


class BnEval16(C.Structure):
    _fields_ = BnEval._fields_


class LaunchPlan(C.Structure):
    _fields_ = [(n, C.c_int) for n in ("family", "mi", "tA", "tB", "pro", "epi", "gather", "c3", "vec", "out_bf16", "wbf",
                                       "nb", "chunks", "empty", "kslice", "seg", "Q", "ntiles", "S", "kper", "mt", "nt")] + \
               [("tiles", C.c_long)] + \
               [(n, C.c_int) for n in ("grid_x", "grid_y", "grid_z", "in_launch", "second", "second_mode")]


PLAN_NONE, PLAN_CGEMM, PLAN_SGEMM, PLAN_SKINNY, PLAN_CGEMM16, PLAN_CONV3_WGRAD, PLAN_WGRAD16_W9, PLAN_WGRAD16_W1 = range(8)
(SECOND_NONE, SECOND_CREDUCE, SECOND_CSTATS1, SECOND_CSTATS2_SLABS, SECOND_CSTATS2_C, SECOND_CREDUCE16, SECOND_CGEMM_REDUCE,
 SECOND_SPLITK_REDUCE) = range(8)


class ImageDesc(C.Structure):
    _fields_ = [("offset", C.c_int64), ("H", C.c_int32), ("W", C.c_int32), ("C", C.c_int32), ("tab_h", C.c_int32),
                ("tab_v", C.c_int32), ("reserved", C.c_int32)]


MAX_BANNED, MAX_NGRAM = 64, 8


class SearchOpts(C.Structure):
    _fields_ = [("min_length", C.c_int32), ("no_repeat_ngram", C.c_int32), ("n_banned", C.c_int32),
                ("banned", C.c_int32 * MAX_BANNED)]


class Diversity(C.Structure):
    _fields_ = [("groups", C.c_int32), ("penalty", C.c_float)]


MAX_REQUIRED = 4


class Constraints(C.Structure):
    _fields_ = [("n_images", C.c_int32), ("pad_token", C.c_int32), ("required", C.c_void_p)]


class SampleFilter(C.Structure):
    _fields_ = [("top_k", C.c_int32), ("top_p", C.c_float)]


_SIGS = {
    "scnattn_version": ([], i32),
# ... 64 lines not shown
                                C.POINTER(Params), vp, i32, i32, i32, vp], i32),
    "scnattn_ensemble_workspace_con": ([i32, C.POINTER(Dims), i32, i32, i32, C.POINTER(SearchOpts), C.POINTER(Constraints),
                                        C.POINTER(sz)], i32),
    "scnattn_ensemble_layout_con": ([i32, C.POINTER(Dims), i32, i32, i32, C.POINTER(SearchOpts), C.POINTER(Constraints),
                                     C.POINTER(i64)], i32),
    "scnattn_ensemble_init_con": ([vp, i32, C.POINTER(Dims), i32, i32, i32, C.POINTER(SearchOpts), C.POINTER(Constraints),
                                   C.POINTER(Params), vp, C.POINTER(vp), i32, vp], i32),
    "scnattn_ensemble_steps_con": ([vp, i32, C.POINTER(Dims), i32, i32, i32, C.POINTER(SearchOpts), C.POINTER(Constraints),
                                    C.POINTER(Params), vp, C.POINTER(f32), i32, i32, i32, i32, vp], i32),
    "scnattn_beam_row_topk_con": ([vp, i32, i32, i32, vp, i64, vp, vp, C.POINTER(SearchOpts), i32, i32, vp, i32, vp, vp, vp,
                                   vp, vp, vp, i32], i32),
    "scnattn_beam_row_topk_ens_con": ([vp, i32, i32, i32, i32, C.POINTER(vp), C.POINTER(i64), C.POINTER(f32), i32, vp, vp,
                                       C.POINTER(SearchOpts), i32, i32, vp, i32, vp, vp, vp, vp, vp, vp, i32], i32),
    "scnattn_beam_merge_banks": ([vp, i32, i32, i32, i32, i32, vp, vp, vp, vp, vp, vp, C.POINTER(vp)], i32),
    "scnattn_rollout_workspace": ([C.POINTER(Dims), i32, i32, i32, C.POINTER(sz)], i32),
    "scnattn_rollout_layout": ([C.POINTER(Dims), i32, i32, i32, C.POINTER(i64)], i32),
    "scnattn_rollout_init": ([vp, C.POINTER(Dims), i32, i32, i32, C.POINTER(Params), vp, vp, i32, vp], i32),
    "scnattn_rollout_steps": ([vp, C.POINTER(Dims), i32, i32, i32, C.POINTER(Params), vp, i32, f32, C.c_uint64, C.c_uint32,
                               i32, i32, i32, vp], i32),
    "scnattn_rollout_pick": ([vp, i32, i32, i32, vp, i64, f32, C.c_uint64, C.c_uint32, i32, i32, i32, i32,
                              C.POINTER(vp)], i32),
    "scnattn_rollout_advance": ([vp, i32, i32, i32, i32, vp, vp, vp, vp, vp], i32),
    "scnattn_rollout_workspace_f": ([C.POINTER(Dims), i32, i32, i32, C.POINTER(SampleFilter), C.POINTER(sz)], i32),
    "scnattn_rollout_layout_f": ([C.POINTER(Dims), i32, i32, i32, C.POINTER(SampleFilter), C.POINTER(i64)], i32),
    "scnattn_rollout_init_f": ([vp, C.POINTER(Dims), i32, i32, i32, C.POINTER(SampleFilter), C.POINTER(Params), vp, vp, i32,
                                vp], i32),
    "scnattn_rollout_steps_f": ([vp, C.POINTER(Dims), i32, i32, i32, C.POINTER(SampleFilter), C.POINTER(Params), vp, i32, f32,
                                 C.c_uint64, C.c_uint32, i32, i32, i32, vp], i32),
    "scnattn_rollout_pick_f": ([vp, i32, i32, i32, vp, i64, f32, C.c_uint64, C.c_uint32, i32, i32, i32, i32, C.POINTER(vp),
                                C.POINTER(SampleFilter), vp, i32], i32),
    "scnattn_rollout_workspace_sc": ([C.POINTER(Dims), i32, i32, i32, C.POINTER(sz)], i32),
    "scnattn_rollout_layout_sc": ([C.POINTER(Dims), i32, i32, i32, C.POINTER(i64)], i32),
    "scnattn_rollout_init_sc": ([vp, C.POINTER(Dims), i32, i32, i32, C.POINTER(Params), vp, vp, i32, vp, i64, vp, vp], i32),
    "scnattn_rollout_steps_sc": ([vp, C.POINTER(Dims), i32, i32, i32, C.POINTER(Params), vp, f32, i32, i32, vp], i32),
    "scnattn_rollout_score": ([vp, i32, i32, i32, vp, i64, f32, i32, i32, C.POINTER(vp), vp, vp, vp], i32),
    "scnattn_sgemm": ([vp, i32, i32, i32, i32, i32, f32, vp, i64, vp, i64, f32, vp, i64, vp, vp, i32, i64, i64, i64], i32),
    "scnattn_sgemm_ws": ([vp, i32, i32, i32, i32, i32, f32, vp, i64, vp, i64, f32, vp, i64, vp, vp, i32, i64, i64, i64,
                          vp, i64], i32),
    "scnattn_cgemm": ([vp, i32, i32, i32, i32, i32, f32, vp, i64, vp, i64, f32, vp, i64, vp, vp, i32, i64, i64, i64,
                       vp, i64, C.POINTER(ConvExtra)], i32),
    "scnattn_cgemm_row_tiles": ([i32], i32),
    "scnattn_conv1x1_fwd": ([vp, i32, i32, i32, vp, vp, vp, C.POINTER(ConvExtra), vp, i64], i32),
    "scnattn_conv1x1_dgrad": ([vp, i32, i32, i32, vp, vp, i32, f32, vp, C.POINTER(ConvExtra), vp, i64], i32),
    "scnattn_conv1x1_wgrad": ([vp, i32, i32, i32, vp, vp, vp, C.POINTER(ConvExtra), vp, i64], i32),
    "scnattn_conv3x3_fwd": ([vp, i32, i32, i32, i32, i32, i32, vp, vp, vp, C.POINTER(ConvExtra), vp, i64], i32),
    "scnattn_conv3x3_dgrad": ([vp, i32, i32, i32, i32, i32, vp, vp, vp, C.POINTER(ConvExtra), vp, i64], i32),
    "scnattn_conv3x3_wgrad": ([vp, i32, i32, i32, i32, i32, i32, vp, vp, vp, vp, i64, i32], i32),
    "scnattn_conv3x3_dgrad_strided": ([vp, i32, i32, i32, i32, i32, i32, vp, vp, vp, vp, i64], i32),
    "scnattn_conv1x1_fwd_bn_eval": ([vp, i32, i32, i32, vp, vp, vp, C.POINTER(BnEval), C.POINTER(ConvExtra), vp, i64], i32),
    "scnattn_conv3x3_fwd_bn_eval": ([vp, i32, i32, i32, i32, i32, i32, vp, vp, vp, C.POINTER(BnEval), C.POINTER(ConvExtra),
                                     vp, i64], i32),
    "scnattn_cgemm_stat_ld": ([i32], i32),
    "scnattn_bn_finalize": ([vp, i64, i32, vp, i32, i32, vp, f32, f32, vp, vp, vp, vp, vp, vp, vp], i32),
    "scnattn_bn_apply_fin": ([vp, i64, i32, vp, vp, i32, vp, i32, i32, vp, f32, f32, vp, vp, i32, vp, vp, vp, vp, vp, vp], i32),
    "scnattn_bn_bwd_reduce": ([vp, i32, i32, vp, vp, vp, i32, vp, vp, i32, vp, i32, vp, C.POINTER(C.c_int)], i32),
    "scnattn_bn_bwd_dx_fin": ([vp, i64, i32, vp, vp, i32, vp, vp, vp, vp, i32, i32, vp, vp, vp], i32),
    "scnattn_bf16_weights": ([vp, i32, vp, vp, i32], i32),
    "scnattn_cgemm16": ([vp, i32, i32, i32, vp, i64, vp, i64, f32, vp, i64, i32, vp, i64, C.POINTER(ConvExtra)], i32),
    "scnattn_conv3x3_fwd16": ([vp, i32, i32, i32, i32, i32, i32, vp, vp, vp, C.POINTER(ConvExtra), vp, i64], i32),
    "scnattn_conv1x1_fwd_bn_eval16": ([vp, i32, i32, i32, vp, vp, vp, C.POINTER(BnEval16), C.POINTER(ConvExtra), vp, i64], i32),
    "scnattn_conv3x3_fwd_bn_eval16": ([vp, i32, i32, i32, i32, i32, i32, vp, vp, vp, C.POINTER(BnEval16), C.POINTER(ConvExtra),
                                       vp, i64], i32),
    "scnattn_conv3x3_dgrad16": ([vp, i32, i32, i32, i32, i32, i32, vp, vp, vp, C.POINTER(ConvExtra), vp, i64], i32),
    "scnattn_wgrad16_3x3": ([vp, i32, i32, i32, i32, i32, vp, vp, vp, vp, i64, i32], i32),
    "scnattn_block16_sizes": ([vp, vp, vp, vp, vp, vp], i32),
    "scnattn_block16_fwd": ([vp, vp], i32),
    "scnattn_block16_bwd": ([vp, vp, vp, vp], i32),
    "scnattn_wgrad16_rows": ([vp, i32, i32, i32, vp, vp, i64, vp, i64, i32, i32, i32, i32, i32, i32, i32, vp, i64, i32], i32),
    "scnattn_stem_tiles": ([i32, i32, i32], i32),
    "scnattn_stem_conv7": ([vp, i32, i32, i32, vp, i64, i64, i64, i64, vp, i64, i64, i64, i64, vp, vp, vp], i32),
    "scnattn_stem_bn_relu_maxpool": ([vp, i32, i32, i32, i32, vp, vp, vp, i32], i32),
    "scnattn_bn_stats_fold": ([vp, i32, i32, vp, f32, f32, vp, vp, vp, vp, vp, vp, vp, vp], i32),
    "scnattn_skinny_gemm": ([vp, i32, i32, i32, i32, vp, i64, i64, vp, i64, i64, vp, i64, i64, i64, i32,
                             C.POINTER(i32)], i32),
    "scnattn_skinny_gemm_bf16w": ([vp, i32, i32, i32, i32, vp, i64, i64, vp, i64, i64, vp, i64, i64, i64, i32,
                                   C.POINTER(i32)], i32),
    "scnattn_skinny_gemm_bf16": ([vp, i32, i32, i32, i32, vp, i64, i64, vp, i64, i64, vp, i64, i64, i64, i32,
                                  C.POINTER(i32)], i32),
    "scnattn_f32_to_bf16": ([vp, i64, vp, vp], i32),
    "scnattn_attn_scores": ([vp, i32, i32, i32, vp, vp, i32, i64, i64, vp, vp, vp, vp, vp], i32),
    "scnattn_attn_context": ([vp, i32, i32, i32, vp, vp, vp, i32, i64, i64, vp, vp, i64, vp, vp, vp, vp], i32),
    "scnattn_mean_pixels": ([vp, i32, i32, i32, vp, vp], i32),
    "scnattn_attn_dalpha": ([vp, i32, i32, i32, vp, vp, vp, i64, vp], i32),
    "scnattn_attn_softmax_bwd": ([vp, i32, i32, i32, vp, vp, vp, vp, vp, vp, vp, i64], i32),
    "scnattn_attn_datt1_post_blocks": ([i32, i32], i32),
    "scnattn_attn_datt1_post": ([vp, i32, i32, i32, i32, vp, vp, vp, vp, vp, vp, vp], i32),
    "scnattn_attn_scores_bf16": ([vp, i32, i32, i32, vp, vp, i32, i64, i64, vp, vp, vp, vp, vp], i32),
    "scnattn_attn_context_bf16": ([vp, i32, i32, i32, vp, vp, vp, i32, i64, i64, vp, vp, i64, vp, vp, vp, vp], i32),
    "scnattn_attn_dalpha_bf16": ([vp, i32, i32, i32, vp, vp, vp, i64, vp], i32),
    "scnattn_attn_softmax_bwd_bf16": ([vp, i32, i32, i32, vp, vp, vp, vp, vp, vp, vp, i64], i32),
    "scnattn_attn_datt1_post_bf16": ([vp, i32, i32, i32, i32, vp, vp, vp, vp, vp, vp, vp], i32),
    "scnattn_attn_context_pooled": ([vp, i32, i32, i32, vp, i32, C.POINTER(Pool), vp, vp, i32, i64, i64, vp, vp, i64, vp, vp,
                                     vp, vp, vp], i32),
    "scnattn_attn_softmax_bwd_pooled": ([vp, i32, i32, i32, vp, i32, vp, vp, vp, C.POINTER(Pool), vp, vp, i64, vp, vp,
                                         i64], i32),
    "scnattn_weighted_rows": ([vp, i32, i32, i32, vp, vp, vp], i32),
    "scnattn_pool_expand": ([vp, i32, i32, i32, C.POINTER(Pool), vp, vp, vp], i32),
    "scnattn_pool_transpose": ([vp, i32, i32, i32, C.POINTER(Pool), vp, vp], i32),
    "scnattn_add_bcast_rows_w": ([vp, i32, i32, i32, vp, vp, vp], i32),
    "scnattn_scn_mix_fwd": ([vp, i32, i32, vp, i32, i64, i64, vp, vp, i32, i64, i64, vp, vp, vp, vp, vp], i32),
    "scnattn_lstm_fwd": ([vp, i32, i32, vp, i32, i64, i64, i64, vp, vp, vp, vp, vp, vp, vp], i32),
    "scnattn_lstm_bwd": ([vp, i32, i32, i32, vp, vp, i32, i64, i64, vp, vp, vp, vp, vp], i32),
    "scnattn_scn_mix_bwd": ([vp, i32, i32, vp, i32, i64, i64, i64, vp, vp, vp, vp, vp, vp, i64, vp, vp], i32),
    "scnattn_gate_bwd": ([vp, i32, i32, vp, i32, i64, i64, vp, vp, vp, vp, i64], i32),
    "scnattn_transpose2d": ([vp, i32, i32, vp, i64, vp, i64], i32),
    "scnattn_colsum": ([vp, i32, i32, vp, i64, vp, f32], i32),
# ... 136 lines not shown
```

indonesian-image-captioning_amd/scnattn/block.py:

```python
from collections import namedtuple

import torch
from torch import nn

PART_FLOATS = 2 << 20

Geom = namedtuple("Geom", "N Cin Hi Wi p C4 s Ho Wo Rin Rout")


def bns(mod):
    m = mod._modules
    d = m.get("downsample")
    return (m["bn1"], m["bn2"], m["bn3"]) + ((d[1],) if d is not None else ())


def convs(mod):
    m = mod._modules
    d = m.get("downsample")
    return (m["conv1"], m["conv2"], m["conv3"]) + ((d[0],) if d is not None else ())


def params(mod):
    p = tuple(t for cv, bn in zip(convs(mod), bns(mod)) for t in (cv.weight, bn.weight, bn.bias))
    return p + (None,) * (12 - len(p))
# ... 27 lines not shown

def structural_reason(mod, x):
    if x.dim() != 4:
        return "input is not an (N, C, H, W) map"
    m, s = mod._modules, mod.stride
    c1, c2, c3, d = m["conv1"], m["conv2"], m["conv3"], m.get("downsample")
    if d is not None and (len(d) != 2 or not isinstance(d[0], nn.Conv2d) or not isinstance(d[1], nn.BatchNorm2d)):
        return "downsample is not a 1x1 convolution at the block's stride + BatchNorm"
    for bn in bns(mod):
        if not bn.affine:
            return "a BatchNorm is not affine"
        if not bn.track_running_stats:
            return "a BatchNorm has no running statistics"
        if mod.training and bn.momentum is None:
            return "a BatchNorm has no momentum (cumulative average)"
    for cv in convs(mod):
        if cv.bias is not None or cv.groups != 1 or cv.dilation != (1, 1):
            return "a convolution has a bias, groups or dilation"
    if (c1.kernel_size, c1.stride, c1.padding) != ((1, 1), (1, 1), (0, 0)) \
            or (c3.kernel_size, c3.stride, c3.padding) != ((1, 1), (1, 1), (0, 0)):
        return "conv1 / conv3 are not 1x1 at stride 1"
    if s not in (1, 2) or (c2.kernel_size, c2.stride, c2.padding) != ((3, 3), (s, s), (1, 1)):
        return "conv2 is not 3x3 / padding 1 at stride 1 or 2"
    p, cin, c4 = c1.out_channels, c1.in_channels, c3.out_channels
    if p % 16 or cin % 16 or c4 % 16:
        return "widths (%d, %d, %d) are not multiples of 16" % (cin, p, c4)
    if x.shape[1] != cin:
        return "input has %d channels, conv1 takes %d" % (x.shape[1], cin)
    if d is not None:
        if (d[0].kernel_size, d[0].stride, d[0].padding, d[0].out_channels) != ((1, 1), (s, s), (0, 0), c4):
            return "downsample is not a 1x1 convolution at the block's stride + BatchNorm"
    elif s != 1 or cin != c4:
        return "no downsample, but the identity does not match the output"
    return None


def reason(mod, x, enabled, training, dtype):
    if not enabled:
        return "fused kernels disabled (scnattn.conv.ENABLED is False)"
    if mod.training != training:
        return "module is in %s mode" % ("training" if mod.training else "eval")
    if dtype == torch.float32 and torch.is_autocast_enabled():
        return "autocast is enabled"
    if not x.is_cuda:
        return "input is not a GPU tensor"
    if x.dtype != dtype:
        return "input is not a %s map" % str(dtype)[6:]
    r = structural_reason(mod, x)
    if r is None and training and any(bn.weight.dtype != torch.float32 for bn in bns(mod)[:3]):
        return "a BatchNorm parameter is not fp32"
    return r


def grads(need, dx, dw, dgb):
    out = [None, dx]
    for w, gb in zip(dw, dgb):
        out += [w, None, None] if gb is None else [w, gb[1], gb[0]]
    return tuple(o if n else None for o, n in zip(out, need))
```

indonesian-image-captioning_amd/scnattn/conv.py:

```python
import ctypes as C
import os

import torch

from . import _lib
from . import block as B
from ._lib import ConvExtra

ENABLED = True
SIDE_WGRAD = True
CONV3 = "hip"
if os.environ.get("SCNATTN_CONV3", "hip") != "hip":
    raise RuntimeError("SCNATTN_CONV3=%s: the MIOpen A/B branch of conv2 is gone (as is round 2's per-shape stopwatch); "
                       "unset the variable or set it to 'hip'" % os.environ["SCNATTN_CONV3"])
W3_SLICES = int(os.environ.get("SCNATTN_W3_SLICES", "0"))

_bufs = {}


def _launch(dev):
    st = torch._C._cuda_getCurrentRawStream(dev.index if dev.index is not None else torch.cuda.current_device())
    b = _bufs.get((dev, st))
    if b is None:
        b = _bufs[(dev, st)] = (torch.empty(16 << 20, device=dev, dtype=torch.float32),
# ... 100 lines not shown
    return ok


def join_side_streams():
    for sd in _sides.values():
        sd.join()


def _chk(rc, what):
    if rc:
        _lib.check(rc, what)


def _as2d(t4):
    n, c, h, w = t4.shape
    return t4.permute(0, 2, 3, 1).reshape(n * h * w, c)


def _as4d(t2, n, h, w):
    return t2.view(n, h, w, t2.shape[1]).permute(0, 3, 1, 2)


def _conv_fwd(h, st, x2, w2, R, Cin, Cout, ws, ex):
    y = torch.empty((R, Cout), device=x2.device, dtype=torch.float32)
    _chk(h.scnattn_conv1x1_fwd(st, R, Cin, Cout, x2.data_ptr(), w2.data_ptr(), y.data_ptr(), C.byref(ex), ws.data_ptr(),
                               ws.numel()), "scnattn_conv1x1_fwd")
    return y


def _shift(bn):
    s = getattr(bn, "_scn_shift", None)
    if s is None or s.device != bn.running_mean.device or s.shape != bn.running_mean.shape:
        s = bn.running_mean.detach().clone()
    return s


def _set_shift(bn, mean):
    bn._scn_shift = mean


def _finalize(h, st, R, Cn, part, bn_mod, shift, gamma, beta, want_ss):
    dev = part.device
    stats = torch.empty((2, Cn), device=dev, dtype=torch.float32)
    ss = torch.empty((Cn, 2), device=dev, dtype=torch.float32) if want_ss else None
    _chk(h.scnattn_bn_finalize(st, R, Cn, part.data_ptr(), h.scnattn_cgemm_stat_ld(R), h.scnattn_cgemm_row_tiles(R),
                               shift.data_ptr(), bn_mod.eps, bn_mod.momentum, stats[0].data_ptr(), stats[1].data_ptr(),
                               bn_mod.running_mean.data_ptr(), bn_mod.running_var.data_ptr(),
                               gamma.data_ptr() if want_ss else None, beta.data_ptr() if want_ss else None,
                               ss.data_ptr() if want_ss else None), "scnattn_bn_finalize")
    _set_shift(bn_mod, stats[0])
    return stats, ss


def _apply_fin(h, st, R, Cn, z, res, part, bn_mod, shift, gamma, beta, relu):
    stats = torch.empty((2, Cn), device=z.device, dtype=torch.float32)
    y = torch.empty_like(z)
    _chk(h.scnattn_bn_apply_fin(st, R, Cn, z.data_ptr(), None if res is None else res.data_ptr(),
                                1 if z.dtype == torch.bfloat16 else 0, part.data_ptr(),
                                h.scnattn_cgemm_stat_ld(R), h.scnattn_cgemm_row_tiles(R), shift.data_ptr(), bn_mod.eps,
                                bn_mod.momentum, gamma.data_ptr(), beta.data_ptr(), 1 if relu else 0, y.data_ptr(),
                                stats[0].data_ptr(), stats[1].data_ptr(), bn_mod.running_mean.data_ptr(),
                                bn_mod.running_var.data_ptr(), None), "scnattn_bn_apply_fin")
    _set_shift(bn_mod, stats[0])
    return y, stats


def _bwd_reduce(h, st, R, Cn, dy, y, z, stats, relu, bnpart, want_g):
    g = torch.empty((R, Cn), device=dy.device, dtype=dy.dtype) if want_g else None
    nch = C.c_int(0)
    _chk(h.scnattn_bn_bwd_reduce(st, R, Cn, dy.data_ptr(), None if y is None else y.data_ptr(), z.data_ptr(),
                                 1 if dy.dtype == torch.bfloat16 else 0, stats[0].data_ptr(), stats[1].data_ptr(), 1 if relu else 0, bnpart.data_ptr(),
                                 bnpart.numel() // (2 * Cn), None if g is None else g.data_ptr(), C.byref(nch)),
         "scnattn_bn_bwd_reduce")
    return g, nch.value


def _bwd_dx_fin(h, st, R, Cn, g, z, stats, gamma, partial, ldp, nchunk, dz):
    dgb = torch.empty((2, Cn), device=g.device, dtype=torch.float32)
    _chk(h.scnattn_bn_bwd_dx_fin(st, R, Cn, g.data_ptr(), z.data_ptr(), 1 if g.dtype == torch.bfloat16 else 0,
                                 stats[0].data_ptr(), stats[1].data_ptr(),
                                 gamma.data_ptr(), partial.data_ptr(), ldp, nchunk, dgb[0].data_ptr(), dgb[1].data_ptr(),
                                 dz.data_ptr()), "scnattn_bn_bwd_dx_fin")
    return dgb


def _grad_out(w):
    gv = getattr(w, "_scn_flat_grad", None)
    task = _sweep_id()
    first = task == -1 or getattr(w, "_scn_sweep", None) != task
    w._scn_sweep = task
    if gv is None or w.grad is not None or not first:
        return torch.empty_like(w)
    return gv.detach()


def _wt(h, st, w, cout, cin):
    wt = torch.empty((cin, cout), device=w.device, dtype=torch.float32)
    _chk(h.scnattn_transpose2d(st, cout, cin, w.data_ptr(), cin, wt.data_ptr(), cout), "scnattn_transpose2d")
    return wt


class _BottleneckFn(torch.autograd.Function):
    @staticmethod
    def forward(ctx, mod, x, w1, g1, b1, w2, g2, b2, w3, g3, b3, wd, gd, bd):
        dev = x.device
        h, st, ws, part, bnpart = _launch(dev)
        x = B.channels_last(x)
        N, Cin, Hi, Wi, p, C4, s, Ho, Wo, Rin, Rout = g = B.geometry(mod, x)
        x2 = _as2d(x)
        bn1, bn2, bn3 = mod.bn1, mod.bn2, mod.bn3
        sh1 = _shift(bn1)
        ex = ConvExtra(epi=1, stat_partial=part.data_ptr(), stat_shift=sh1.data_ptr())
        z1 = _conv_fwd(h, st, x2, w1.view(p, Cin), Rin, Cin, p, ws, ex)
        a1, st1 = _apply_fin(h, st, Rin, p, z1, None, part, bn1, sh1, g1, b1, True)
        sh2 = _shift(bn2)
        z2 = torch.empty((Rout, p), device=dev, dtype=torch.float32)
        ex3 = ConvExtra(epi=1, stat_partial=part.data_ptr(), stat_shift=sh2.data_ptr())
        _chk(h.scnattn_conv3x3_fwd(st, N, Hi, Wi, p, p, s, a1.data_ptr(), w2.data_ptr(), z2.data_ptr(), C.byref(ex3),
                                   ws.data_ptr(), ws.numel()), "scnattn_conv3x3_fwd")
        st2, ss2 = _finalize(h, st, Rout, p, part, bn2, sh2, g2, b2, True)
        sh3 = _shift(bn3)
        ex = ConvExtra(pro=1, epi=1, pro_ss=ss2.data_ptr(), stat_partial=part.data_ptr(), stat_shift=sh3.data_ptr())
        z3 = _conv_fwd(h, st, z2, w3.view(C4, p), Rout, p, C4, ws, ex)
        zd = std = None
        if wd is not None:
            bnd = mod.downsample[1]
            shd = _shift(bnd)
            ex = ConvExtra(epi=1, stat_partial=bnpart.data_ptr(), stat_shift=shd.data_ptr(),
                           stride=s, Hi=Hi, Wi=Wi, Ho=Ho, Wo=Wo)
            zd = _conv_fwd(h, st, x2, wd.view(C4, Cin), Rout, Cin, C4, ws, ex)
            idn, std = _apply_fin(h, st, Rout, C4, zd, None, bnpart, bnd, shd, gd, bd, False)
        else:
            idn = x2
        out, st3 = _apply_fin(h, st, Rout, C4, z3, idn, part, bn3, sh3, g3, b3, True)
        wt = wt_ev = None
        if ctx.needs_input_grad[1] and SIDE_WGRAD:
            sd = _side(dev)
            wt = torch.empty((Cin, p), device=dev, dtype=torch.float32)
            sw = sd.fork(torch.cuda.current_stream(dev), w1, wt)
            _chk(h.scnattn_transpose2d(sw, p, Cin, w1.data_ptr(), Cin, wt.data_ptr(), p), "scnattn_transpose2d")
            wt_ev = torch.cuda.Event()
            wt_ev.record(sd.stream)
        ctx.wt, ctx.wt_ev, ctx.geom = wt, wt_ev, g
        ctx.save_for_backward(x, w1, g1, b1, w2, g2, b2, w3, g3, b3, wd, gd, bd, z1, a1, z2, z3, out, zd, st1, st2, ss2,
                              st3, std)
        return _as4d(out, N, Ho, Wo)

    @staticmethod
    def backward(ctx, dout):
        (x, w1, g1, b1, w2, g2, b2, w3, g3, b3, wd, gd, bd, z1, a1, z2, z3, out, zd, st1, st2, ss2, st3,
         std) = ctx.saved_tensors
        N, Cin, Hi, Wi, p, C4, s, Ho, Wo, Rin, Rout = ctx.geom
        dev = x.device
        h, st, ws, part, bnpart = _launch(dev)
        need = ctx.needs_input_grad
        dout2 = _as2d(B.channels_last(dout.float()))
        x2 = _as2d(x)
        f32 = dict(device=dev, dtype=torch.float32)
        ld_out, nc_out = h.scnattn_cgemm_stat_ld(Rout), h.scnattn_cgemm_row_tiles(Rout)
        ld_in, nc_in = h.scnattn_cgemm_stat_ld(Rin), h.scnattn_cgemm_row_tiles(Rin)
        dres, nch = _bwd_reduce(h, st, Rout, C4, dout2, out, z3, st3, True, bnpart, True)
        dz3 = torch.empty((Rout, C4), **f32)
        dgb3 = _bwd_dx_fin(h, st, Rout, C4, dres, z3, st3, g3, bnpart, (nch + 3) & ~3, nch, dz3)
        main = torch.cuda.current_stream(dev)
        side = _side(dev) if side_ok(w1, w2, w3, wd) else None
        dw3 = None
        if need[8]:
            dw3 = _grad_out(w3)
            ex = ConvExtra(pro=2, pro_ss=ss2.data_ptr())
            sw, wsw = (side.fork(main, dz3, z2, ss2, dw3), side.ws) if side else (st, ws)
            _chk(h.scnattn_conv1x1_wgrad(sw, Rout, p, C4, dz3.data_ptr(), z2.data_ptr(), dw3.data_ptr(), C.byref(ex),
                                         wsw.data_ptr(), wsw.numel()), "scnattn_conv1x1_wgrad")
        dz2 = torch.empty((Rout, p), **f32)
        ex = ConvExtra(epi=2, stat_partial=part.data_ptr(), ez=z2.data_ptr(), emean=st2[0].data_ptr(),
                       einvstd=st2[1].data_ptr(), egamma=g2.data_ptr(), ebeta=b2.data_ptr(), ldz=p,
                       pro_ss=ss2.data_ptr())
        _chk(h.scnattn_conv1x1_dgrad(st, Rout, p, C4, dz3.data_ptr(), w3.data_ptr(), 0, 0.0, dz2.data_ptr(), C.byref(ex),
                                     ws.data_ptr(), ws.numel()), "scnattn_conv1x1_dgrad")
        dgb2 = _bwd_dx_fin(h, st, Rout, p, dz2, z2, st2, g2, part, ld_out, nc_out, dz2)
        dw2 = None
        dz1 = torch.empty((Rin, p), **f32)
        if need[5]:
            dw2 = _grad_out(w2)
            sw, wsw = (side.fork(main, dz2, a1, dw2), side.ws) if side else (st, ws)
            _chk(h.scnattn_conv3x3_wgrad(sw, N, Hi, Wi, p, p, s, dz2.data_ptr(), a1.data_ptr(), dw2.data_ptr(),
                                         wsw.data_ptr(), wsw.numel(), W3_SLICES), "scnattn_conv3x3_wgrad")
        if s == 1:
            ex = ConvExtra(epi=2, stat_partial=part.data_ptr(), ez=z1.data_ptr(), emean=st1[0].data_ptr(),
                           einvstd=st1[1].data_ptr(), egamma=g1.data_ptr(), ebeta=b1.data_ptr(), ldz=p)
            _chk(h.scnattn_conv3x3_dgrad(st, N, Hi, Wi, p, p, dz2.data_ptr(), w2.data_ptr(), dz1.data_ptr(), C.byref(ex),
                                         ws.data_ptr(), ws.numel()), "scnattn_conv3x3_dgrad")
            dgb1 = _bwd_dx_fin(h, st, Rin, p, dz1, z1, st1, g1, part, ld_in, nc_in, dz1)
        else:
            da1 = torch.empty((Rin, p), **f32)
            _chk(h.scnattn_conv3x3_dgrad_strided(st, N, Hi, Wi, p, p, s, dz2.data_ptr(), w2.data_ptr(), da1.data_ptr(),
                                                 ws.data_ptr(), ws.numel()), "scnattn_conv3x3_dgrad_strided")
            g1m, nch = _bwd_reduce(h, st, Rin, p, da1, a1, z1, st1, True, bnpart, True)
            dgb1 = _bwd_dx_fin(h, st, Rin, p, g1m, z1, st1, g1, bnpart, (nch + 3) & ~3, nch, dz1)
            del g1m, da1
        need_dx = need[1]
        dw1 = None
        if need[2]:
            dw1 = _grad_out(w1)
            sw, wsw = (side.fork(main, dz1, x, dw1), side.ws) if side else (st, ws)
            ex1 = ConvExtra()
            _chk(h.scnattn_conv1x1_wgrad(sw, Rin, Cin, p, dz1.data_ptr(), x2.data_ptr(), dw1.data_ptr(), C.byref(ex1),
                                         wsw.data_ptr(), wsw.numel()), "scnattn_conv1x1_wgrad")
        wt = ctx.wt
        if need_dx:
            if wt is None:
                wt = _wt(h, st, w1, p, Cin)
            else:
                main.wait_event(ctx.wt_ev)
        dwd = dgbd = None
        dx = None
        if wd is not None:
            _, nch = _bwd_reduce(h, st, Rout, C4, dres, None, zd, std, False, bnpart, False)
            dzd = torch.empty((Rout, C4), **f32)
            dgbd = _bwd_dx_fin(h, st, Rout, C4, dres, zd, std, gd, bnpart, (nch + 3) & ~3, nch, dzd)
            if need[11]:
                dwd = _grad_out(wd)
                ex = ConvExtra(stride=s, Hi=Hi, Wi=Wi, Ho=Ho, Wo=Wo)
                sw, wsw = (side.fork(main, dzd, x, dwd), side.ws) if side else (st, ws)
                _chk(h.scnattn_conv1x1_wgrad(sw, Rout, Cin, C4, dzd.data_ptr(), x2.data_ptr(), dwd.data_ptr(),
                                             C.byref(ex), wsw.data_ptr(), wsw.numel()), "scnattn_conv1x1_wgrad")
            if need_dx:
                dx = torch.empty((Rin, Cin), **f32)
                _chk(h.scnattn_conv1x1_dgrad(st, Rin, Cin, p, dz1.data_ptr(), wt.data_ptr(), 1, 0.0,
                                             dx.data_ptr(), None, ws.data_ptr(), ws.numel()), "scnattn_conv1x1_dgrad")
                dxd = torch.empty((Rout, Cin), **f32)
                _chk(h.scnattn_conv1x1_dgrad(st, Rout, Cin, C4, dzd.data_ptr(), wd.data_ptr(), 0, 0.0, dxd.data_ptr(), None,
                                             ws.data_ptr(), ws.numel()), "scnattn_conv1x1_dgrad")
                dx.view(N, Hi, Wi, Cin)[:, ::s, ::s].add_(dxd.view(N, Ho, Wo, Cin))
        elif need_dx:
            dx = dres
            _chk(h.scnattn_conv1x1_dgrad(st, Rin, Cin, p, dz1.data_ptr(), wt.data_ptr(), 1, 1.0,
                                         dx.data_ptr(), None, ws.data_ptr(), ws.numel()), "scnattn_conv1x1_dgrad")
        if side:
            side.mark()
        dx4 = _as4d(dx, N, Hi, Wi) if dx is not None else None
        return B.grads(need, dx4, (dw1, dw2, dw3, dwd), (dgb1, dgb2, dgb3, dgbd))


def train_reason(mod, x):
    r = B.reason(mod, x, ENABLED, True, torch.float32)
    if r:
        return r
    g = B.geometry(mod, x)
    if g.p % 32 if g.s == 1 else g.p % 128 or g.Hi % 2 or g.Wi % 2:
        return "conv2's width / map parity is not one the 3x3 kernels address"
    if not mod.conv2.weight.is_contiguous(memory_format=torch.channels_last):
        return "conv2's weight is not channels-last"
    if B.part_floats(g) > B.PART_FLOATS:
        return "statistics partials exceed the scratch"
    return None


def usable(mod, x):
    return train_reason(mod, x) is None


def bottleneck(mod, x):
    B.bump_counters(B.bns(mod))
    return _BottleneckFn.apply(mod, x, *B.params(mod))
```

indonesian-image-captioning_amd/scnattn/resnet.py:

```python
import os

import torch
from torch import nn

from . import block as B


def configure_miopen():
    os.environ.setdefault("MIOPEN_FIND_MODE", "2")
    os.environ.setdefault("MIOPEN_LOG_LEVEL", "3")


class FusedBatchNorm2d(nn.BatchNorm2d):

    counter_managed = False
    use_fused = True

    def forward(self, x, residual=None, relu=False):
        if not x.is_cuda or not FusedBatchNorm2d.use_fused or self.weight is None or not self.track_running_stats or self.momentum is None:
            y = super().forward(x)
            if residual is not None:
                y = y + residual
            return torch.relu(y) if relu else y
        from . import functional as SF
        if self.training:
            B.bump_counters((self,))
        return SF.bn_act(x, residual, self.weight, self.bias, self.running_mean, self.running_var, self.training,
                         self.momentum, self.eps, relu)


class Bottleneck(nn.Module):
    expansion = 4

    def __init__(self, inplanes, planes, stride=1, downsample=None):
        super().__init__()
        self.conv1 = nn.Conv2d(inplanes, planes, kernel_size=1, bias=False)
        self.bn1 = FusedBatchNorm2d(planes)
        self.conv2 = nn.Conv2d(planes, planes, kernel_size=3, stride=stride, padding=1, bias=False)
        self.bn2 = FusedBatchNorm2d(planes)
        self.conv3 = nn.Conv2d(planes, planes * self.expansion, kernel_size=1, bias=False)
        self.bn3 = FusedBatchNorm2d(planes * self.expansion)
        self.relu = nn.ReLU(inplace=True)
        self.downsample = downsample
        self.stride = stride

    def forward(self, x):
        from . import conv as _conv, conv_eval as _ce, conv16 as _c16, conv_eval16 as _ce16
        if _conv.usable(self, x):
            return _conv.bottleneck(self, x)
        if _ce.eval_reason(self, x) is None:
            return _ce.bottleneck_eval(self, x)
        if _c16.usable(self, x):
            return _c16.bottleneck(self, x)
        if _ce16.eval16_reason(self, x) is None:
            return _ce16.bottleneck_eval16(self, x)
        return self.module_forward(x)

    def module_forward(self, x):
        identity = x if self.downsample is None else self.downsample(x)
        out = self.bn1(self.conv1(x), relu=True)
        out = self.bn2(self.conv2(out), relu=True)
        return self.bn3(self.conv3(out), residual=identity, relu=True)


def manage_bn_counters(trunk):
    bns = [m for m in trunk.modules() if isinstance(m, FusedBatchNorm2d) and m.num_batches_tracked is not None]
    if not bns:
        return None
    dev = bns[0].num_batches_tracked.device
    flat = torch.zeros(len(bns), dtype=torch.long, device=dev)
    for i, m in enumerate(bns):
        flat[i] = m.num_batches_tracked.to(dev)
        m._buffers["num_batches_tracked"] = flat[i]
        m.counter_managed = True
    return flat


def _make_layer(inplanes, planes, blocks, stride):
    downsample = None
    if stride != 1 or inplanes != planes * Bottleneck.expansion:
        downsample = nn.Sequential(
            nn.Conv2d(inplanes, planes * Bottleneck.expansion, kernel_size=1, stride=stride, bias=False),
            FusedBatchNorm2d(planes * Bottleneck.expansion))
    layers = [Bottleneck(inplanes, planes, stride, downsample)]
    inplanes = planes * Bottleneck.expansion
    for _ in range(1, blocks):
        layers.append(Bottleneck(inplanes, planes))
    return nn.Sequential(*layers), inplanes


def resnet152_trunk(depths=(3, 8, 36, 3), keep_avgpool=False):
    mods = [nn.Conv2d(3, 64, kernel_size=7, stride=2, padding=3, bias=False), FusedBatchNorm2d(64),
            nn.ReLU(inplace=True), nn.MaxPool2d(kernel_size=3, stride=2, padding=1)]
    inplanes = 64
    for planes, blocks, stride in zip((64, 128, 256, 512), depths, (1, 2, 2, 2)):
        layer, inplanes = _make_layer(inplanes, planes, blocks, stride)
        mods.append(layer)
    if keep_avgpool:
        mods.append(nn.AdaptiveAvgPool2d((1, 1)))
    trunk = nn.Sequential(*mods)
    for m in trunk.modules():
        if isinstance(m, nn.Conv2d):
# ... 6 lines not shown
```

indonesian-image-captioning_amd/scnattn/stem.py:

```python
import torch

from . import _lib
from . import block as B
from . import conv as _conv


def stem_reason(trunk, x):
    if not (_conv.ENABLED and x.is_cuda and x.dtype == torch.float32 and x.dim() == 4):
        return "not an fp32 (N, C, H, W) GPU batch, or fused kernels disabled"
    if torch.is_autocast_enabled() and torch.get_autocast_dtype("cuda") != torch.bfloat16:
        return "autocast to a dtype other than bf16"
    if len(trunk) < 4:
        return "fewer than four children"
    c1, bn, pool = trunk[0], trunk[1], trunk[3]
    if not (isinstance(c1, torch.nn.Conv2d) and isinstance(bn, torch.nn.BatchNorm2d) and isinstance(pool, torch.nn.MaxPool2d)):
        return "children are not conv, BatchNorm, _, max-pool"
    if c1.weight.shape != (64, 3, 7, 7) or c1.stride != (2, 2) or c1.padding != (3, 3) or c1.dilation != (1, 1) \
            or c1.bias is not None or c1.groups != 1 or c1.weight.dtype != torch.float32 or x.shape[1] != 3:
        return "conv1 is not the 7x7 / 2 convolution of 3 fp32 channels to 64"
    if bn.weight is None or bn.running_mean is None or (bn.training and bn.momentum is None):
        return "bn1 is not affine with running statistics"
    ks, sd, pd = (v if isinstance(v, tuple) else (v, v) for v in (pool.kernel_size, pool.stride, pool.padding))
    if ks != (3, 3) or sd != (2, 2) or pd != (1, 1) or pool.dilation not in (1, (1, 1)) or pool.ceil_mode:
        return "the pool is not the 3x3 / 2 max-pool"
    if torch.is_grad_enabled() and (x.requires_grad or c1.weight.requires_grad or bn.weight.requires_grad or bn.bias.requires_grad):
        return "the stem needs a gradient"
    return None


def usable(trunk, x):
    return stem_reason(trunk, x) is None


def stem(trunk, x, bf16=False):
    c1, bn = trunk[0], trunk[1]
    h = _lib.lib()
    dev = x.device
    st = torch._C._cuda_getCurrentRawStream(dev.index)
    N, _, H, W = x.shape
    Hz, Wz = (H - 1) // 2 + 1, (W - 1) // 2 + 1
    Hp, Wp = (Hz - 1) // 2 + 1, (Wz - 1) // 2 + 1
    w = c1.weight
    z = torch.empty((N * Hz * Wz, 64), device=dev, dtype=torch.float32)
    ss = torch.empty((64, 2), device=dev, dtype=torch.float32)
    if bn.training:
        B.bump_counters((bn,))
        nt = h.scnattn_stem_tiles(N, H, W)
        ldp = (nt + 3) & ~3
        part = torch.empty((2, 64, ldp), device=dev, dtype=torch.float32)
        stats = torch.empty((2, 64), device=dev, dtype=torch.float32)
        shift = _conv._shift(bn)
        _conv._chk(h.scnattn_stem_conv7(st, N, H, W, x.data_ptr(), *x.stride(), w.data_ptr(), *w.stride(), z.data_ptr(),
                                        part.data_ptr(), shift.data_ptr()), "scnattn_stem_conv7")
        _conv._chk(h.scnattn_bn_finalize(st, N * Hz * Wz, 64, part.data_ptr(), ldp, nt, shift.data_ptr(), bn.eps,
                                         bn.momentum, stats[0].data_ptr(), stats[1].data_ptr(),
                                         bn.running_mean.data_ptr(), bn.running_var.data_ptr(), bn.weight.data_ptr(),
                                         bn.bias.data_ptr(), ss.data_ptr()), "scnattn_bn_finalize")
        _conv._set_shift(bn, stats[0])
    else:
        _conv._chk(h.scnattn_stem_conv7(st, N, H, W, x.data_ptr(), *x.stride(), w.data_ptr(), *w.stride(), z.data_ptr(),
                                        None, None), "scnattn_stem_conv7")
        with torch.no_grad():
            sc = bn.weight * torch.rsqrt(bn.running_var + bn.eps)
            ss.copy_(torch.stack([sc, bn.bias - bn.running_mean * sc], dim=1))
    out = torch.empty((N * Hp * Wp, 64), device=dev, dtype=torch.bfloat16 if bf16 else torch.float32)
    _conv._chk(h.scnattn_stem_bn_relu_maxpool(st, N, Hz, Wz, 64, z.data_ptr(), ss.data_ptr(), out.data_ptr(), 1 if bf16 else 0),
               "scnattn_stem_bn_relu_maxpool")
    return out.view(N, Hp, Wp, 64).permute(0, 3, 1, 2)


def run_trunk(trunk, x, drop_last=0):
    fused = usable(trunk, x)
    bf16 = torch.is_autocast_enabled() and torch.get_autocast_dtype("cuda") == torch.bfloat16
    if bf16 and (fused or getattr(trunk, "_scn_w16", None) is not None):
        from . import conv16 as _c16
        _c16.refresh_weights(trunk)
    children = list(trunk.children())
    children = children[:len(children) - drop_last]
    if fused:
        y = stem(trunk, x, bf16)
        for child in children[4:]:
            y = child(y)
        return y
    if not drop_last:
        return trunk(x)
    for child in children:
        x = child(x)
    return x
```

Baseline: 813.7 images/sec.

## Defer bottleneck BN3+residual+ReLU into next block's conv1 GEMM prologue

```diff
diff --git a/include/scnattn.h b/include/scnattn.h
--- a/include/scnattn.h
+++ b/include/scnattn.h
@@ -433,6 +433,7 @@
     int stride, Hi, Wi, Ho, Wo;
     int force_split;
     int force_mi;
+    const float* idn; const float* pro_tab; float* out;
 } scnattn_conv_extra;
 int scnattn_cgemm(void* stream, int transA, int transB, int M, int N, int K, float alpha, const float* A, long lda,
                   const float* B, long ldb, float beta, float* C, long ldc, const float* bias, const float* rowmask,
@@ -473,6 +474,9 @@
 int scnattn_bn_finalize(void* stream, long R, int C, const float* partial, int ldp, int nchunk, const float* shift,
                         float eps, float momentum, float* mean, float* invstd, float* run_mean, float* run_var,
                         const float* gamma, const float* beta, float* ss_out);
+int scnattn_bn_finalize_tab(void* stream, long R, int C, const float* partial, int ldp, int nchunk, const float* shift,
+                            float eps, float momentum, float* mean, float* invstd, float* run_mean, float* run_var,
+                            const float* gamma, const float* beta, float* tab_out);
 int scnattn_bn_apply_fin(void* stream, long R, int C, const void* z, const void* res, int bf16, const float* partial, int ldp,
                          int nchunk, const float* shift, float eps, float momentum, const float* gamma, const float* beta,
                          int relu, void* y, float* mean, float* invstd, float* run_mean, float* run_var, float* ss_out);
diff --git a/indonesian-image-captioning_amd/csrc/api.cpp b/indonesian-image-captioning_amd/csrc/api.cpp
--- a/indonesian-image-captioning_amd/csrc/api.cpp
+++ b/indonesian-image-captioning_amd/csrc/api.cpp
@@ -549,6 +549,7 @@
     x.ez = e->ez; x.emean = e->emean; x.einvstd = e->einvstd; x.egamma = e->egamma; x.ebeta = e->ebeta; x.ldz = e->ldz;
     x.stride = e->stride < 1 ? 1 : e->stride; x.Hi = e->Hi; x.Wi = e->Wi; x.Ho = e->Ho; x.Wo = e->Wo;
     x.force_split = e->force_split; x.force_mi = e->force_mi;
+    x.idn = e->idn; x.pro_tab = e->pro_tab; x.out = e->out;
     return x;
 }
 
@@ -566,7 +567,7 @@
 int scnattn_conv1x1_fwd(void* stream, int R, int Cin, int Cout, const float* x, const float* w, float* y,
                         const scnattn_conv_extra* ex, float* ws, long ws_floats) {
     const ConvExtra e = to_extra(ex);
-    SCN_ARG(!ex || ex->pro != 2, "conv1x1_fwd: prologue must be on the input (pro = 1)");
+    SCN_ARG(!ex || ex->pro != 2, "conv1x1_fwd: prologue must be on the input (pro = 1 or 3)");
     return cgemm(ST(stream), false, true, R, Cout, Cin, 1.f, x, Cin, w, Cin, 0.f, y, Cout, nullptr, nullptr, 1, 0, 0, 0,
                  ws, ws ? ws_floats : 0, ex ? &e : nullptr);
 }
@@ -697,6 +698,14 @@
                          beta, ss_out);
 }
 
+int scnattn_bn_finalize_tab(void* stream, long R, int C, const float* partial, int ldp, int nchunk, const float* shift,
+                            float eps, float momentum, float* mean, float* invstd, float* run_mean, float* run_var,
+                            const float* gamma, const float* beta, float* tab_out) {
+    SCN_ARG(tab_out, "bn_finalize_tab: tab_out is NULL");
+    return bn_finalize_t(ST(stream), R, C, partial, ldp, nchunk, shift, eps, momentum, mean, invstd, run_mean, run_var, gamma,
+                         beta, nullptr, tab_out);
+}
+
 int scnattn_bn_apply_fin(void* stream, long R, int C, const void* z, const void* res, int bf16, const float* partial, int ldp,
                          int nchunk, const float* shift, float eps, float momentum, const float* gamma, const float* beta,
                          int relu, void* y, float* mean, float* invstd, float* run_mean, float* run_var, float* ss_out) {
diff --git a/indonesian-image-captioning_amd/csrc/batchnorm.hip b/indonesian-image-captioning_amd/csrc/batchnorm.hip
--- a/indonesian-image-captioning_amd/csrc/batchnorm.hip
+++ b/indonesian-image-captioning_amd/csrc/batchnorm.hip
@@ -262,6 +262,7 @@
 struct BnFin {
     const float* partial; int ldp, nchunk; const float* shift; float eps, momentum;
     float* mean; float* invstd; float* run_mean; float* run_var; float* ss_out;
+    float* tab_out;
 };
 
 template <typename T, bool RELU, bool RES>
@@ -364,6 +365,7 @@
         f.ss_out[2 * c] = sc;
         f.ss_out[2 * c + 1] = fmaf(-mu, sc, beta[c]);
     }
+    if (f.tab_out) *reinterpret_cast<f32x4*>(f.tab_out + 4 * c) = f32x4{mu, is, gamma[c], beta[c]};
 }
 
 template <typename T>
@@ -604,12 +606,13 @@
 
 int bn_finalize_t(hipStream_t st, long R, int C, const float* partial, int ldp, int nchunk, const float* shift, float eps,
                   float momentum, float* mean, float* invstd, float* run_mean, float* run_var, const float* gamma,
-                  const float* beta, float* ss_out) {
+                  const float* beta, float* ss_out, float* tab_out) {
     SCN_ARG(R > 0 && C > 0 && partial && ldp >= nchunk && ldp % 4 == 0 && nchunk > 0 && mean && invstd && aligned16(partial),
             "bn_finalize_t: bad argument");
     SCN_ARG(!ss_out || (gamma && beta), "bn_finalize_t: folded scale/shift need gamma and beta");
+    SCN_ARG(!tab_out || (gamma && beta && aligned16(tab_out)), "bn_finalize_t: the constants table needs gamma, beta and 16-byte alignment");
     SCN_ARG(2L * C * ldp * 4 < 0x7fffffffL, "bn_finalize_t: partial too large");
-    BnFin f{partial, ldp, nchunk, shift, eps, momentum, mean, invstd, run_mean, run_var, ss_out};
+    BnFin f{partial, ldp, nchunk, shift, eps, momentum, mean, invstd, run_mean, run_var, ss_out, tab_out};
     hipLaunchKernelGGL(bn_finalize_t_kernel, dim3(cdiv(C, 64)), dim3(256), 0, st, R, C, gamma, beta, f);
     SCN_LAUNCH_CHECK();
     return 0;
diff --git a/indonesian-image-captioning_amd/csrc/cgemm.hip b/indonesian-image-captioning_amd/csrc/cgemm.hip
--- a/indonesian-image-captioning_amd/csrc/cgemm.hip
+++ b/indonesian-image-captioning_amd/csrc/cgemm.hip
@@ -27,6 +27,7 @@
     int mt, nt;
     ConvGeom geo;
     const float* pro_ss;
+    const float* idn; const float* pro_tab; float* out;
     float* stat_partial; const float* stat_shift;
     int ldp;
     const float* ez; const float* emean; const float* einvstd; const float* egamma; const float* ebeta;
@@ -38,12 +39,16 @@
 
 template <int MI, bool A_MC, bool B_MC, int PRO, int EPI, bool GATHER, bool VEC, int C3 = 0>
 __global__ __launch_bounds__(256, MI == 2 ? 2 : 3) void cgemm_kernel(CArgs g) {
-    __shared__ __attribute__((aligned(16))) float lds[NSTAGE * STAGE_F];
     constexpr bool W41 = (MI == 4);
     constexpr int RB = W41 ? 1 : MI;
     constexpr int TM = W41 ? 128 : 64 * MI;
     constexpr int ACH = TM / 64;
-    constexpr int LPT = ACH + 2 + (PRO == 1 ? 1 : 0);
+    constexpr bool APRO = PRO == 1 || PRO == 3;
+    constexpr int LPT = ACH + 2 + (PRO == 1 ? 1 : PRO == 3 ? ACH + 1 : 0);
+    static_assert(PRO != 3 || (!A_MC && !GATHER && C3 == 0 && !W41), "PRO 3: plain k-contiguous A rows, 64- or 128-row tiles");
+    constexpr int SF = STAGE_F + ((PRO == 3 && TM == 128) ? TILE_F : 0);
+    constexpr int IOFF = TM == 128 ? STAGE_F : TM * TK;
+    __shared__ __attribute__((aligned(16))) float lds[NSTAGE * SF];
 
     const int tid = threadIdx.x, lane = tid & 63, wave = tid >> 6;
     const int wm = W41 ? wave : wave >> 1, wn = W41 ? 0 : wave & 1;
@@ -70,7 +75,9 @@
                                 : ((long)(g.N - 1) * g.ldb + g.K);
     const __amdgpu_buffer_rsrc_t ars = make_rsrc(A, (unsigned)(a_elems * 4));
     const __amdgpu_buffer_rsrc_t brs = make_rsrc(B, (unsigned)(b_elems * 4));
-    const __amdgpu_buffer_rsrc_t srs = make_rsrc(g.pro_ss, PRO == 1 ? (unsigned)g.K * 8u : 0u);
+    const __amdgpu_buffer_rsrc_t srs = make_rsrc(PRO == 3 ? g.pro_tab : g.pro_ss, PRO == 1 ? (unsigned)g.K * 8u : PRO == 3 ? (unsigned)g.K * 16u : 0u);
+    const __amdgpu_buffer_rsrc_t irs = make_rsrc(g.idn, PRO == 3 ? (unsigned)(a_elems * 4) : 0u);
+    const __amdgpu_buffer_rsrc_t qrs = make_rsrc(g.out, (PRO == 3 && tn == 0) ? (unsigned)(a_elems * 4) : 0u);
 
     unsigned a_off[ACH], b_off[2];
     bool a_ok[ACH], b_ok[2];
@@ -120,7 +127,7 @@
 
     auto issue_piece = [&](int kt, int stage, auto pc) {
         constexpr int P = decltype(pc)::value;
-        float* sa = lds + stage * STAGE_F;
+        float* sa = lds + stage * SF;
         float* sb = sa + TILE_F;
         const int k0 = kbeg + kt * TK;
         if constexpr (P < ACH) {
@@ -184,6 +191,21 @@
             const int kk = k0 + (lane >> 1);
             dma4(srs, sx, (lane < 32 && kk < Kend) ? (unsigned)(2 * k0 + lane) * 4u : OOB_OFF);
         }
+        if constexpr (PRO == 3 && P >= ACH + 2 && P < 2 * ACH + 2) {
+            constexpr int c = P - ACH - 2;
+            const int chunk = wave * ACH + c;
+            const int kk = k0 + 4 * ((lane & 3) ^ (((chunk * 16 + (lane >> 2)) >> 2) & 3));
+            dma16(irs, sa + IOFF + chunk * 256, (a_ok[c] && kk < Kend) ? a_off[c] + (unsigned)k0 * 4u : OOB_OFF);
+        }
+        if constexpr (PRO == 3 && P == 2 * ACH + 2) {
+            float* sx = sa + 2 * TILE_F + wave * 64;
+            dma4(srs, sx, (k0 + (lane >> 2) < Kend) ? (unsigned)(4 * k0 + lane) * 4u : OOB_OFF);
+        }
+    };
+    auto out_granule = [&](int kt, int c) -> unsigned {
+        const int chunk = wave * ACH + c, k0 = kbeg + kt * TK;
+        const int kk = k0 + 4 * ((lane & 3) ^ (((chunk * 16 + (lane >> 2)) >> 2) & 3));
+        return (a_ok[c] && kk < Kend) ? a_off[c] + (unsigned)k0 * 4u : OOB_OFF;
     };
 
     auto issue = [&](int kt, int stage) {
@@ -192,6 +214,9 @@
         if constexpr (LPT > 2) issue_piece(kt, stage, std::integral_constant<int, 2>{});
         if constexpr (LPT > 3) issue_piece(kt, stage, std::integral_constant<int, 3>{});
         if constexpr (LPT > 4) issue_piece(kt, stage, std::integral_constant<int, 4>{});
+        if constexpr (LPT > 5) issue_piece(kt, stage, std::integral_constant<int, 5>{});
+        if constexpr (LPT > 6) issue_piece(kt, stage, std::integral_constant<int, 6>{});
+        static_assert(LPT <= 7, "more DMA pieces than issue() sends");
     };
 
     f32x16 acc[RB][2];
@@ -214,7 +239,7 @@
     }
 
     auto prologue_in_lds = [&](int stg) {
-        float* sa = lds + stg * STAGE_F;
+        float* sa = lds + stg * SF;
         const float* sx = sa + 2 * TILE_F + wave * 64;
 #pragma unroll
         for (int c = 0; c < ACH; ++c) {
@@ -222,6 +247,19 @@
             const int row = chunk * 16 + (lane >> 2), gsrc = (lane & 3) ^ ((row >> 2) & 3);
             float* p = sa + chunk * 256 + lane * 4;
             f32x4 v = *reinterpret_cast<f32x4*>(p);
+            if constexpr (PRO == 3) {
+                const f32x4 r = *reinterpret_cast<const f32x4*>(sa + IOFF + chunk * 256 + lane * 4);
+#pragma unroll
+                for (int q = 0; q < 4; ++q) {
+                    const f32x4 t = *reinterpret_cast<const f32x4*>(sx + 16 * gsrc + 4 * q);
+                    float y = bn_norm(v[q], t[0], t[1], t[2], t[3]);
+                    y += r[q];
+                    v[q] = fmaxf(y, 0.f);
+                }
+                *reinterpret_cast<f32x4*>(p) = v;
+                buf_store4(qrs, out_granule(stg, c), v);
+                continue;
+            }
             const f32x4 t0 = *reinterpret_cast<const f32x4*>(sx + 8 * gsrc), t1 = *reinterpret_cast<const f32x4*>(sx + 8 * gsrc + 4);
             v[0] = fmaxf(fmaf(v[0], t0[0], t0[1]), 0.f);
             v[1] = fmaxf(fmaf(v[1], t0[2], t0[3]), 0.f);
@@ -234,7 +272,7 @@
 
     auto load_piece = [&](int stg, auto pc, float (&a)[RB][8], float (&b)[2][8]) {
         constexpr int P = decltype(pc)::value;
-        const float* sa = lds + stg * STAGE_F;
+        const float* sa = lds + stg * SF;
         const float* sb = sa + TILE_F;
         if constexpr (P < RB) {
             constexpr int i = P;
@@ -272,24 +310,44 @@
     };
     auto slot = [](int kt) { return kt % NSTAGE; };
     [[maybe_unused]] f32x4 pv[ACH], pt0[ACH], pt1[ACH];
+    [[maybe_unused]] f32x4 pr[ACH], pt2[ACH], pt3[ACH];
     auto pro_read = [&](int stg) {
-        const float* sa = lds + stg * STAGE_F;
+        const float* sa = lds + stg * SF;
         const float* sx = sa + 2 * TILE_F + wave * 64;
 #pragma unroll
         for (int c = 0; c < ACH; ++c) {
             const int chunk = wave * ACH + c;
             const int row = chunk * 16 + (lane >> 2), gsrc = (lane & 3) ^ ((row >> 2) & 3);
             pv[c] = *reinterpret_cast<const f32x4*>(sa + chunk * 256 + lane * 4);
+            if constexpr (PRO == 3) {
+                pr[c] = *reinterpret_cast<const f32x4*>(sa + IOFF + chunk * 256 + lane * 4);
+                pt0[c] = *reinterpret_cast<const f32x4*>(sx + 16 * gsrc);
+                pt1[c] = *reinterpret_cast<const f32x4*>(sx + 16 * gsrc + 4);
+                pt2[c] = *reinterpret_cast<const f32x4*>(sx + 16 * gsrc + 8);
+                pt3[c] = *reinterpret_cast<const f32x4*>(sx + 16 * gsrc + 12);
+                continue;
+            }
             pt0[c] = *reinterpret_cast<const f32x4*>(sx + 8 * gsrc);
             pt1[c] = *reinterpret_cast<const f32x4*>(sx + 8 * gsrc + 4);
         }
     };
-    auto pro_apply = [&](int stg) {
-        float* sa = lds + stg * STAGE_F;
+    auto pro_apply = [&](int stg, int kt) {
+        float* sa = lds + stg * SF;
 #pragma unroll
         for (int c = 0; c < ACH; ++c) {
             const int chunk = wave * ACH + c;
             f32x4 v = pv[c];
+            if constexpr (PRO == 3) {
+                float y0 = bn_norm(v[0], pt0[c][0], pt0[c][1], pt0[c][2], pt0[c][3]);
+                float y1 = bn_norm(v[1], pt1[c][0], pt1[c][1], pt1[c][2], pt1[c][3]);
+                float y2 = bn_norm(v[2], pt2[c][0], pt2[c][1], pt2[c][2], pt2[c][3]);
+                float y3 = bn_norm(v[3], pt3[c][0], pt3[c][1], pt3[c][2], pt3[c][3]);
+                y0 += pr[c][0]; y1 += pr[c][1]; y2 += pr[c][2]; y3 += pr[c][3];
+                v = f32x4{fmaxf(y0, 0.f), fmaxf(y1, 0.f), fmaxf(y2, 0.f), fmaxf(y3, 0.f)};
+                *reinterpret_cast<f32x4*>(sa + chunk * 256 + lane * 4) = v;
+                buf_store4(qrs, out_granule(kt, c), v);
+                continue;
+            }
             v[0] = fmaxf(fmaf(v[0], pt0[c][0], pt0[c][1]), 0.f);
             v[1] = fmaxf(fmaf(v[1], pt0[c][2], pt0[c][3]), 0.f);
             v[2] = fmaxf(fmaf(v[2], pt1[c][0], pt1[c][1]), 0.f);
@@ -298,20 +356,20 @@
         }
     };
     constexpr int NPL = RB + 2, NM = 16 * RB;
-    constexpr int NPC = NPL + LPT + (PRO == 1 ? 2 : 0);
+    constexpr int NPC = NPL + LPT + (APRO ? 2 : 0);
     float fa0[RB][8], fb0[2][8], fa1[RB][8], fb1[2][8];
     auto kstep = [&](int kt, float (&ac)[RB][8], float (&bc)[2][8], float (&an)[RB][8], float (&bn)[2][8]) {
         const int s_next = slot(kt + 1), s_dma = slot(kt), s_pro = slot(kt + 2);
         auto piece = [&](auto pc) {
             constexpr int P = decltype(pc)::value;
-            if constexpr (PRO != 1) {
+            if constexpr (!APRO) {
                 if constexpr (P < NPL) load_piece(s_next, pc, an, bn);
                 else if constexpr (P < NPC) issue_piece(kt + 3, s_dma, std::integral_constant<int, P - NPL>{});
             } else {
                 if constexpr (P < LPT) issue_piece(kt + 3, s_dma, pc);
                 else if constexpr (P == LPT) { wait_vmcnt<LPT>(); pro_read(s_pro); }
                 else if constexpr (P < LPT + 1 + NPL) load_piece(s_next, std::integral_constant<int, P - LPT - 1>{}, an, bn);
-                else if constexpr (P < NPC) pro_apply(s_pro);
+                else if constexpr (P < NPC) pro_apply(s_pro, kt + 2);
             }
         };
         if (PRO == 2) {
@@ -339,10 +397,12 @@
                     if (m == 8 * NM / NPC) piece(std::integral_constant<int, 8>{});
                     if (m == 9 * NM / NPC) piece(std::integral_constant<int, 9>{});
                     if (m == 10 * NM / NPC) piece(std::integral_constant<int, 10>{});
+                    if (m == 11 * NM / NPC) piece(std::integral_constant<int, 11>{});
+                    if (m == 12 * NM / NPC) piece(std::integral_constant<int, 12>{});
                     __builtin_amdgcn_sched_barrier(0);
                 }
-        static_assert(NPC <= 11 && NPC <= NM, "more pieces than slots");
-        if (PRO != 1) wait_vmcnt<LPT>();
+        static_assert(NPC <= 13 && NPC <= NM, "more pieces than slots");
+        if (!APRO) wait_vmcnt<LPT>();
         __builtin_amdgcn_s_waitcnt(0xC07F);
         __builtin_amdgcn_s_barrier();
     };
@@ -351,11 +411,11 @@
     issue(1, 1);
     issue(2, 2);
     asm volatile("s_waitcnt vmcnt(%0)" :: "n"(2 * LPT) : "memory");
-    if (PRO == 1) prologue_in_lds(0);
+    if (APRO) prologue_in_lds(0);
     __builtin_amdgcn_s_barrier();
     load_frags(0, fa0, fb0);
     wait_vmcnt<LPT>();
-    if (PRO == 1) prologue_in_lds(1);
+    if (APRO) prologue_in_lds(1);
     __builtin_amdgcn_s_waitcnt(0xC07F);
     __builtin_amdgcn_s_barrier();
     for (int kt = 0; kt < nk; kt += 2) {
@@ -978,7 +1038,12 @@
 
 template <int MI>
 void launch_layout(hipStream_t st, dim3 grid, const CArgs& g, const LaunchPlan& p) {
-    if (!p.tA && p.tB) {
+    if (p.pro == 3) {
+        if constexpr (MI != 4) {
+            if (p.epi == 1) hipLaunchKernelGGL((cgemm_kernel<MI, false, false, 3, 1, false, true>), grid, dim3(256), 0, st, g);
+            else            hipLaunchKernelGGL((cgemm_kernel<MI, false, false, 3, 0, false, true>), grid, dim3(256), 0, st, g);
+        }
+    } else if (!p.tA && p.tB) {
         if (p.gather) { if (p.pro == 1) launch_ev<MI, false, false, 1, true>(st, grid, g, p); else launch_ev<MI, false, false, 0, true>(st, grid, g, p); }
         else          { if (p.pro == 1) launch_ev<MI, false, false, 1, false>(st, grid, g, p); else launch_ev<MI, false, false, 0, false>(st, grid, g, p); }
     } else if (!p.tA && !p.tB) {
@@ -1004,7 +1069,7 @@
     int mi = 2;
     if ((long)cdiv(M, 128) * cdiv(N, TN) * batch < 256 && M > 64 && c3 != 1 && c3 != 2 && c3 != 4) mi = 1;
     if (c3 == 4 && (long)cdiv(M, 128) * cdiv(N, TN) * 4 < 768) mi = 1;
-    if (N <= 64 && M >= 128 && c3 != 3) mi = 4;
+    if (N <= 64 && M >= 128 && c3 != 3 && f.pro != 3) mi = 4;
     if (g_cgemm_mi == 1 || g_cgemm_mi == 2) mi = g_cgemm_mi;
     if (f.force_mi > 0) mi = f.force_mi;
     SCN_ARG(mi == 1 || mi == 2 || (mi == 4 && c3 != 3), "cgemm: bad tile selector");
@@ -1057,6 +1122,8 @@
     SCN_ARG(epi != 3 || S == 1 || in_launch, "cgemm: eval BatchNorm epilogue of a split product needs the in-launch combine");
     const int kepi = (S > 1 && !in_launch) ? 0 : (epi_in ? epi : 0);
     if (c3) SCN_ARG(f.vec, "cgemm: 3x3 mode needs 16-byte row stores");
+    else if (f.pro == 3) SCN_ARG(!tA && tB && !f.gather && f.vec && (mi == 1 || mi == 2) && (kepi == 0 || kepi == 1) && batch == 1,
+                                 "cgemm: the residual prologue takes a plain forward product (64- or 128-row tiles, 16-byte row stores)");
     else if (!tA && !tB) SCN_ARG(!f.gather && f.pro == 0, "cgemm: NN product takes no gather / prologue");
     else if (tA && !tB) SCN_ARG(kepi == 0, "cgemm: TN product takes no statistics epilogue");
     else if (tA && tB) SCN_ARG(!f.gather && f.pro == 0 && kepi == 0, "cgemm: TT product is plain");
@@ -1095,7 +1162,11 @@
                 (c3 == 3 && tA && !tB && N == 9 * ex->c3c && ex->c3c % 128 == 0), "cgemm: 3x3 mode / layout / channel multiple");
         SCN_ARG(ex->c3_src_rows * (c3 == 3 ? ldb : lda) * 4 < 0x7fffffffL, "cgemm: 3x3 source map exceeds the descriptor range");
     }
-    SCN_ARG(pro == 0 || (pro == 1 && !tA) || (pro == 2 && !tB && tA), "cgemm: prologue / layout mismatch");
+    SCN_ARG(pro == 0 || (pro == 1 && !tA) || (pro == 2 && !tB && tA) || (pro == 3 && !tA && tB && !c3), "cgemm: prologue / layout mismatch");
+    SCN_ARG(pro != 3 || (ex->idn && ex->out && ex->pro_tab && aligned16(ex->idn) && aligned16(ex->out) && aligned16(ex->pro_tab) &&
+                         ex->stride <= 1 && (epi == 0 || epi == 1) && beta == 0.f && !bias && !rowmask && batch == 1 &&
+                         (const float*)ex->out != A && ex->out != C && ex->idn != C),
+            "cgemm: residual prologue arguments");
     SCN_ARG(epi == 0 || (batch == 1 && beta == 0.f && !bias && !rowmask && (epi == 3 || ex->stat_partial)),
             "cgemm: statistics epilogue needs a plain product");
     SCN_ARG(epi != 3 || (!tA && tB && pro == 0 && (c3 == 0 || c3 == 1)), "cgemm: eval BatchNorm epilogue: forward products only");
@@ -1106,7 +1177,7 @@
             "cgemm: eval BatchNorm epilogue arguments");
     SCN_ARG(epi != 2 || (ex->ez && ex->emean && ex->einvstd && (ex->pro_ss || (ex->egamma && ex->ebeta)) && ex->ldz % 4 == 0),
             "cgemm: mask epilogue arguments");
-    SCN_ARG(pro == 0 || ex->pro_ss, "cgemm: prologue table");
+    SCN_ARG(pro == 0 || pro == 3 || ex->pro_ss, "cgemm: prologue table");
     SCN_ARG(!gather || (ex->Hi > 0 && ex->Wi > 0 && ex->Ho > 0 && ex->Wo > 0 && batch == 1), "cgemm: gather geometry");
     const bool vec = N % 4 == 0 && ldc % 4 == 0 && sC % 4 == 0 && aligned16(C) &&
                      ((long)(M - 1) * ldc + N) * 4 < 0x7fffffffL && (long)M * N * 4 < 0x7fffffffL;
@@ -1127,6 +1198,7 @@
     if (ex) {
         g.geo = conv_geom(*ex);
         g.pro_ss = ex->pro_ss;
+        g.idn = ex->idn; g.pro_tab = ex->pro_tab; g.out = ex->out;
         g.stat_partial = ex->stat_partial; g.stat_shift = ex->stat_shift; g.ldp = cgemm_stat_ld(M);
         g.ez = ex->ez; g.emean = ex->emean; g.einvstd = ex->einvstd; g.egamma = ex->egamma; g.ebeta = ex->ebeta; g.ldz = ex->ldz;
         g.evar = ex->evar; g.eeps = ex->eeps; g.erelu = ex->erelu;
diff --git a/indonesian-image-captioning_amd/csrc/kernels.h b/indonesian-image-captioning_amd/csrc/kernels.h
--- a/indonesian-image-captioning_amd/csrc/kernels.h
+++ b/indonesian-image-captioning_amd/csrc/kernels.h
@@ -39,6 +39,7 @@
     int c3c = 0;
     long c3_src_rows = 0;
     const float* evar = nullptr; float eeps = 0.f; int erelu = 0;
+    const float* idn = nullptr; const float* pro_tab = nullptr; float* out = nullptr;
 };
 bool cgemm_supported(bool tA, bool tB, int M, int N, int K, const float* A, long lda, const float* B, long ldb,
                      long sA, long sB);
@@ -288,7 +289,7 @@
 
 int bn_finalize_t(hipStream_t st, long R, int C, const float* partial, int ldp, int nchunk, const float* shift, float eps,
                   float momentum, float* mean, float* invstd, float* run_mean, float* run_var, const float* gamma,
-                  const float* beta, float* ss_out);
+                  const float* beta, float* ss_out, float* tab_out = nullptr);
 int bn_apply_fin(hipStream_t st, long R, int C, const void* z, const void* res, int bf16, const float* partial, int ldp, int nchunk,
                  const float* shift, float eps, float momentum, const float* gamma, const float* beta, int relu, void* y,
                  float* mean, float* invstd, float* run_mean, float* run_var, float* ss_out);
diff --git a/indonesian-image-captioning_amd/scnattn/_lib.py b/indonesian-image-captioning_amd/scnattn/_lib.py
--- a/indonesian-image-captioning_amd/scnattn/_lib.py
+++ b/indonesian-image-captioning_amd/scnattn/_lib.py
@@ -44,7 +44,8 @@
                 ("stat_partial", C.c_void_p), ("stat_shift", C.c_void_p), ("ez", C.c_void_p), ("emean", C.c_void_p),
                 ("einvstd", C.c_void_p), ("egamma", C.c_void_p), ("ebeta", C.c_void_p), ("ldz", C.c_long),
                 ("stride", C.c_int), ("Hi", C.c_int), ("Wi", C.c_int), ("Ho", C.c_int), ("Wo", C.c_int),
-                ("force_split", C.c_int), ("force_mi", C.c_int)]
+                ("force_split", C.c_int), ("force_mi", C.c_int),
+                ("idn", C.c_void_p), ("pro_tab", C.c_void_p), ("out", C.c_void_p)]
 
 
 class BnEval(C.Structure):
@@ -215,6 +216,7 @@
                                      vp, i64], i32),
     "scnattn_cgemm_stat_ld": ([i32], i32),
     "scnattn_bn_finalize": ([vp, i64, i32, vp, i32, i32, vp, f32, f32, vp, vp, vp, vp, vp, vp, vp], i32),
+    "scnattn_bn_finalize_tab": ([vp, i64, i32, vp, i32, i32, vp, f32, f32, vp, vp, vp, vp, vp, vp, vp], i32),
     "scnattn_bn_apply_fin": ([vp, i64, i32, vp, vp, i32, vp, i32, i32, vp, f32, f32, vp, vp, i32, vp, vp, vp, vp, vp, vp], i32),
     "scnattn_bn_bwd_reduce": ([vp, i32, i32, vp, vp, vp, i32, vp, vp, i32, vp, i32, vp, C.POINTER(C.c_int)], i32),
     "scnattn_bn_bwd_dx_fin": ([vp, i64, i32, vp, vp, i32, vp, vp, vp, vp, i32, i32, vp, vp, vp], i32),
diff --git a/indonesian-image-captioning_amd/scnattn/block.py b/indonesian-image-captioning_amd/scnattn/block.py
--- a/indonesian-image-captioning_amd/scnattn/block.py
+++ b/indonesian-image-captioning_amd/scnattn/block.py
@@ -103,6 +103,27 @@
     return r
 
 
+def pending(t):
+    return getattr(t, "_scn_pending", None)
+
+
+def set_pending(t, rec):
+    t._scn_pending = rec
+
+
+def clear_pending(t):
+    if getattr(t, "_scn_pending", None) is not None:
+        t._scn_pending = None
+
+
+def materialize(t):
+    rec = pending(t)
+    if rec is not None:
+        rec.fill()
+        t._scn_pending = None
+    return t
+
+
 def grads(need, dx, dw, dgb):
     out = [None, dx]
     for w, gb in zip(dw, dgb):
diff --git a/indonesian-image-captioning_amd/scnattn/conv.py b/indonesian-image-captioning_amd/scnattn/conv.py
--- a/indonesian-image-captioning_amd/scnattn/conv.py
+++ b/indonesian-image-captioning_amd/scnattn/conv.py
@@ -176,6 +176,52 @@
     return stats, ss
 
 
+def _finalize_tab(h, st, R, Cn, part, bn_mod, shift, gamma, beta):
+    dev = part.device
+    stats = torch.empty((2, Cn), device=dev, dtype=torch.float32)
+    tab = torch.empty((Cn, 4), device=dev, dtype=torch.float32)
+    _chk(h.scnattn_bn_finalize_tab(st, R, Cn, part.data_ptr(), h.scnattn_cgemm_stat_ld(R), h.scnattn_cgemm_row_tiles(R),
+                                   shift.data_ptr(), bn_mod.eps, bn_mod.momentum, stats[0].data_ptr(), stats[1].data_ptr(),
+                                   bn_mod.running_mean.data_ptr(), bn_mod.running_var.data_ptr(), gamma.data_ptr(),
+                                   beta.data_ptr(), tab.data_ptr()), "scnattn_bn_finalize_tab")
+    _set_shift(bn_mod, stats[0])
+    return stats, tab
+
+
+DEFER_MIN_ELEMS = int(os.environ.get("SCNATTN_DEFER_MIN_ELEMS", str(1 << 24)))
+
+
+def defer_policy(rows, channels):
+    return rows * channels >= DEFER_MIN_ELEMS
+
+
+def prologue_covers(rows, cout):
+    return cout > 64 or rows < 128
+
+
+class Pending:
+    __slots__ = ("out", "z3", "idn", "stats", "gamma", "beta", "tab", "R", "Cn", "stream")
+
+    def __init__(self, out, z3, idn, stats, gamma, beta, tab, stream):
+        self.out, self.z3, self.idn, self.stats, self.tab, self.stream = out, z3, idn, stats, tab, stream
+        self.gamma, self.beta = gamma.detach(), beta.detach()
+        self.R, self.Cn = out.shape
+
+    def feeds(self, x):
+        dev = x.device
+        return (x.is_cuda and x.dtype == torch.float32 and x.dim() == 4 and x.shape[1] == self.Cn
+                and x.numel() == self.R * self.Cn and x.data_ptr() == self.out.data_ptr()
+                and x.is_contiguous(memory_format=torch.channels_last)
+                and torch._C._cuda_getCurrentRawStream(dev.index if dev.index is not None else torch.cuda.current_device()) == self.stream)
+
+    def fill(self):
+        dev = self.out.device
+        st = torch._C._cuda_getCurrentRawStream(dev.index if dev.index is not None else torch.cuda.current_device())
+        _chk(_lib.lib().scnattn_bn_apply(st, self.R, self.Cn, self.z3.data_ptr(), self.idn.data_ptr(), 0, self.stats[0].data_ptr(),
+                                         self.stats[1].data_ptr(), self.gamma.data_ptr(), self.beta.data_ptr(), 1,
+                                         self.out.data_ptr()), "scnattn_bn_apply")
+
+
 def _apply_fin(h, st, R, Cn, z, res, part, bn_mod, shift, gamma, beta, relu):
     stats = torch.empty((2, Cn), device=z.device, dtype=torch.float32)
     y = torch.empty_like(z)
@@ -226,7 +272,7 @@
 
 class _BottleneckFn(torch.autograd.Function):
     @staticmethod
-    def forward(ctx, mod, x, w1, g1, b1, w2, g2, b2, w3, g3, b3, wd, gd, bd):
+    def forward(ctx, mod, x, w1, g1, b1, w2, g2, b2, w3, g3, b3, wd, gd, bd, pend=None, hold=None):
         dev = x.device
         h, st, ws, part, bnpart = _launch(dev)
         x = B.channels_last(x)
@@ -234,8 +280,13 @@
         x2 = _as2d(x)
         bn1, bn2, bn3 = mod.bn1, mod.bn2, mod.bn3
         sh1 = _shift(bn1)
-        ex = ConvExtra(epi=1, stat_partial=part.data_ptr(), stat_shift=sh1.data_ptr())
-        z1 = _conv_fwd(h, st, x2, w1.view(p, Cin), Rin, Cin, p, ws, ex)
+        if pend is None:
+            ex = ConvExtra(epi=1, stat_partial=part.data_ptr(), stat_shift=sh1.data_ptr())
+            z1 = _conv_fwd(h, st, x2, w1.view(p, Cin), Rin, Cin, p, ws, ex)
+        else:
+            ex = ConvExtra(pro=3, epi=1, stat_partial=part.data_ptr(), stat_shift=sh1.data_ptr(), idn=pend.idn.data_ptr(),
+                           pro_tab=pend.tab.data_ptr(), out=x2.data_ptr())
+            z1 = _conv_fwd(h, st, pend.z3, w1.view(p, Cin), Rin, Cin, p, ws, ex)
         a1, st1 = _apply_fin(h, st, Rin, p, z1, None, part, bn1, sh1, g1, b1, True)
         sh2 = _shift(bn2)
         z2 = torch.empty((Rout, p), device=dev, dtype=torch.float32)
@@ -256,7 +307,12 @@
             idn, std = _apply_fin(h, st, Rout, C4, zd, None, bnpart, bnd, shd, gd, bd, False)
         else:
             idn = x2
-        out, st3 = _apply_fin(h, st, Rout, C4, z3, idn, part, bn3, sh3, g3, b3, True)
+        if hold is None:
+            out, st3 = _apply_fin(h, st, Rout, C4, z3, idn, part, bn3, sh3, g3, b3, True)
+        else:
+            st3, tab = _finalize_tab(h, st, Rout, C4, part, bn3, sh3, g3, b3)
+            out = torch.empty((Rout, C4), device=dev, dtype=torch.float32)
+            hold.append(Pending(out, z3, idn, st3, g3, b3, tab, st))
         wt = wt_ev = None
         if ctx.needs_input_grad[1] and SIDE_WGRAD:
             sd = _side(dev)
@@ -363,7 +419,7 @@
         if side:
             side.mark()
         dx4 = _as4d(dx, N, Hi, Wi) if dx is not None else None
-        return B.grads(need, dx4, (dw1, dw2, dw3, dwd), (dgb1, dgb2, dgb3, dgbd))
+        return B.grads(need, dx4, (dw1, dw2, dw3, dwd), (dgb1, dgb2, dgb3, dgbd)) + (None, None)
 
 
 def train_reason(mod, x):
@@ -384,6 +440,16 @@
     return train_reason(mod, x) is None
 
 
-def bottleneck(mod, x):
+def bottleneck(mod, x, defer_out=False):
     B.bump_counters(B.bns(mod))
-    return _BottleneckFn.apply(mod, x, *B.params(mod))
+    pend = B.pending(x)
+    if pend is not None and not (pend.feeds(x) and prologue_covers(pend.R, mod._modules["conv1"].out_channels)):
+        B.materialize(x)
+        pend = None
+    hold = [] if defer_out else None
+    y = _BottleneckFn.apply(mod, x, *B.params(mod), pend, hold)
+    if pend is not None:
+        B.clear_pending(x)
+    if hold:
+        B.set_pending(y, hold[0])
+    return y
diff --git a/indonesian-image-captioning_amd/scnattn/resnet.py b/indonesian-image-captioning_amd/scnattn/resnet.py
--- a/indonesian-image-captioning_amd/scnattn/resnet.py
+++ b/indonesian-image-captioning_amd/scnattn/resnet.py
@@ -44,10 +44,11 @@
         self.downsample = downsample
         self.stride = stride
 
-    def forward(self, x):
+    def forward(self, x, defer_out=False):
         from . import conv as _conv, conv_eval as _ce, conv16 as _c16, conv_eval16 as _ce16
         if _conv.usable(self, x):
-            return _conv.bottleneck(self, x)
+            return _conv.bottleneck(self, x, defer_out)
+        B.materialize(x)
         if _ce.eval_reason(self, x) is None:
             return _ce.bottleneck_eval(self, x)
         if _c16.usable(self, x):
diff --git a/indonesian-image-captioning_amd/scnattn/stem.py b/indonesian-image-captioning_amd/scnattn/stem.py
--- a/indonesian-image-captioning_amd/scnattn/stem.py
+++ b/indonesian-image-captioning_amd/scnattn/stem.py
@@ -69,6 +69,65 @@
     return out.view(N, Hp, Wp, 64).permute(0, 3, 1, 2)
 
 
+def _Bottleneck():
+    from .resnet import Bottleneck
+    return Bottleneck
+
+
+def _blocks(children):
+    out = []
+    for ch in children:
+        if type(ch) is torch.nn.Sequential and len(ch) and all(isinstance(m, _Bottleneck()) for m in ch) \
+                and not (ch._forward_hooks or ch._forward_pre_hooks):
+            out.extend(ch)
+        else:
+            out.append(ch)
+    return out
+
+
+class MapSpec:
+
+    def __init__(self, shape, dtype, device):
+        self.shape, self.dtype, self.device = torch.Size(shape), dtype, torch.device(device)
+        self.is_cuda = self.device.type == "cuda"
+
+    def dim(self):
+        return len(self.shape)
+
+
+def defer_reason(block, nxt, x):
+    if nxt is None:
+        return "last block of the trunk"
+    if not isinstance(nxt, _Bottleneck()):
+        return "the next module is not a Bottleneck"
+    if x.dim() != 4:
+        return "input is not an (N, C, H, W) map"
+    g = B.geometry(block, x)
+    if not _conv.defer_policy(g.Rout, g.C4):
+        return "the policy keeps the stand-alone pass for a [%d][%d] map" % (g.Rout, g.C4)
+    r = _conv.train_reason(block, x)
+    if r:
+        return "this block: " + r
+    r = _conv.train_reason(nxt, MapSpec((g.N, g.C4, g.Ho, g.Wo), torch.float32, x.device))
+    if r:
+        return "the next block: " + r
+    if not _conv.prologue_covers(g.Rout, nxt._modules["conv1"].out_channels):
+        return "the next conv1 is a 64-column product: the prologue has no instance in its wave layout"
+    if nxt._modules["conv1"].weight.device != block._modules["conv1"].weight.device:
+        return "the next block is on another device"
+    return None
+
+
+def run_blocks(mods, y):
+    for i, m in enumerate(mods):
+        nxt = mods[i + 1] if i + 1 < len(mods) else None
+        if isinstance(m, _Bottleneck()):
+            y = m(y, defer_out=defer_reason(m, nxt, y) is None)
+        else:
+            y = m(B.materialize(y))
+    return B.materialize(y)
+
+
 def run_trunk(trunk, x, drop_last=0):
     fused = usable(trunk, x)
     bf16 = torch.is_autocast_enabled() and torch.get_autocast_dtype("cuda") == torch.bfloat16
@@ -79,9 +138,7 @@
     children = children[:len(children) - drop_last]
     if fused:
         y = stem(trunk, x, bf16)
-        for child in children[4:]:
-            y = child(y)
-        return y
+        return run_blocks(_blocks(children[4:]), y)
     if not drop_last:
         return trunk(x)
     for child in children:
```

Measured after the change: 817.9 images/sec, median of 6. Within noise of the previous version (+0.5%).
